# consilience-dev/llm-map-reduce-summarizer

Measured on AMD Instinct MI355X. Metric: chunks/sec (whole node) + end-to-end wall-clock, 10h transcript, Llama-3-8B, higher is better.
Workload: dtype bf16

## Files before the change

### llm_map_reduce_summarizer_amd/csrc/kernels/norm.hip

```cpp
#include "common.h"

template <int VPT, bool ADD, int Q8 = 0>
__global__ __launch_bounds__(256) void rmsnorm_kernel(const bf16* __restrict__ x, bf16* __restrict__ residual,
                                                      const bf16* __restrict__ w, bf16* __restrict__ out,
                                                      int D, int x_stride, int out_stride, float eps,
                                                      float* __restrict__ qscale = nullptr) {
    __shared__ float red[16];
    const int row = blockIdx.x;
    const int nvec = D >> 3;
    const uint4* xr = reinterpret_cast<const uint4*>(x + (size_t)row * x_stride);
    uint4* rr = ADD ? reinterpret_cast<uint4*>(residual + (size_t)row * D) : nullptr;
    float v[VPT][8];
    const uint4* wr = reinterpret_cast<const uint4*>(w);
    uint4 wv[VPT];
#pragma unroll
    for (int i = 0; i < VPT; ++i) wv[i] = wr[min((int)threadIdx.x + i * 256, nvec - 1)];
    float ss = 0.f;
#pragma unroll
    for (int i = 0; i < VPT; ++i) {
        const int c = threadIdx.x + i * 256;
        if (c < nvec) {
            unpack8(xr[c], v[i]);
            if (ADD) {
                float r[8];
                unpack8(rr[c], r);
#pragma unroll
                for (int j = 0; j < 8; ++j) v[i][j] = (float)(bf16)(v[i][j] + r[j]);
                rr[c] = pack8(v[i]);
            }
#pragma unroll
            for (int j = 0; j < 8; ++j) ss += v[i][j] * v[i][j];
        }
    }
    ss = block_sum(ss, red);
    const float inv = rsqrtf(ss / (float)D + eps);
    float amax = 0.f;
#pragma unroll
    for (int i = 0; i < VPT; ++i) {
        const int c = threadIdx.x + i * 256;
        if (c < nvec) {
            float wf[8];
            unpack8(wv[i], wf);
#pragma unroll
            for (int j = 0; j < 8; ++j) v[i][j] = v[i][j] * inv * wf[j];
            if constexpr (Q8) {
#pragma unroll
                for (int j = 0; j < 8; ++j) amax = fmaxf(amax, fabsf(v[i][j]));
            } else {
                reinterpret_cast<uint4*>(out + (size_t)row * out_stride)[c] = pack8(v[i]);
            }
        }
    }
    if constexpr (Q8) {
        amax = wave_max(amax);
        __syncthreads();
        if ((threadIdx.x & 63) == 0) red[threadIdx.x >> 6] = amax;
        __syncthreads();
        amax = fmaxf(fmaxf(red[0], red[1]), fmaxf(red[2], red[3]));
        const float sc = fmaxf(amax, 1e-12f) / 448.f, qi = 1.f / sc;
        if (threadIdx.x == 0) qscale[row] = sc;
        uint2* qr = reinterpret_cast<uint2*>(reinterpret_cast<uint8_t*>(out) + (size_t)row * out_stride);
#pragma unroll
        for (int i = 0; i < VPT; ++i) {
            const int c = threadIdx.x + i * 256;
            if (c < nvec) {
                float y[8];
#pragma unroll
                for (int j = 0; j < 8; ++j) y[j] = v[i][j] * qi;
                int lo = 0, hi = 0;
                lo = __builtin_amdgcn_cvt_pk_fp8_f32(y[0], y[1], lo, false);
                lo = __builtin_amdgcn_cvt_pk_fp8_f32(y[2], y[3], lo, true);
                hi = __builtin_amdgcn_cvt_pk_fp8_f32(y[4], y[5], hi, false);
                hi = __builtin_amdgcn_cvt_pk_fp8_f32(y[6], y[7], hi, true);
                qr[c] = make_uint2((unsigned)lo, (unsigned)hi);
                if constexpr (Q8 == 2) {
                    float r[8];
                    const auto a0 = __builtin_amdgcn_cvt_pk_f32_fp8(lo, false), a1 = __builtin_amdgcn_cvt_pk_f32_fp8(lo, true);
                    const auto b0 = __builtin_amdgcn_cvt_pk_f32_fp8(hi, false), b1 = __builtin_amdgcn_cvt_pk_f32_fp8(hi, true);
                    r[0] = (y[0] - a0[0]) * 16.f; r[1] = (y[1] - a0[1]) * 16.f;
                    r[2] = (y[2] - a1[0]) * 16.f; r[3] = (y[3] - a1[1]) * 16.f;
                    r[4] = (y[4] - b0[0]) * 16.f; r[5] = (y[5] - b0[1]) * 16.f;
                    r[6] = (y[6] - b1[0]) * 16.f; r[7] = (y[7] - b1[1]) * 16.f;
                    int l2 = 0, h2 = 0;
                    l2 = __builtin_amdgcn_cvt_pk_fp8_f32(r[0], r[1], l2, false);
                    l2 = __builtin_amdgcn_cvt_pk_fp8_f32(r[2], r[3], l2, true);
                    h2 = __builtin_amdgcn_cvt_pk_fp8_f32(r[4], r[5], h2, false);
                    h2 = __builtin_amdgcn_cvt_pk_fp8_f32(r[6], r[7], h2, true);
                    qr[nvec + c] = make_uint2((unsigned)l2, (unsigned)h2);
                }
            }
        }
    }
}

template <bool ADD, int Q8 = 0>
static int launch_rmsnorm(const void* x, void* residual, const void* w, void* out, int T, int D, int x_stride,
                          int out_stride, float eps, hipStream_t s, float* qscale = nullptr) {
    if (T <= 0) return 0;
    if (D % 8 || D > 256 * 8 * 8 || (Q8 && !qscale)) return (int)hipErrorInvalidValue;
    const int vpt = ceil_div(D / 8, 256);
    dim3 g(T), b(256);
    auto X = (const bf16*)x; auto R = (bf16*)residual; auto W = (const bf16*)w; auto O = (bf16*)out;
    if (vpt <= 1) rmsnorm_kernel<1, ADD, Q8><<<g, b, 0, s>>>(X, R, W, O, D, x_stride, out_stride, eps, qscale);
    else if (vpt <= 2) rmsnorm_kernel<2, ADD, Q8><<<g, b, 0, s>>>(X, R, W, O, D, x_stride, out_stride, eps, qscale);
    else if (vpt <= 4) rmsnorm_kernel<4, ADD, Q8><<<g, b, 0, s>>>(X, R, W, O, D, x_stride, out_stride, eps, qscale);
    else rmsnorm_kernel<8, ADD, Q8><<<g, b, 0, s>>>(X, R, W, O, D, x_stride, out_stride, eps, qscale);
    return (int)hipGetLastError();
}

MRSUM_API int mrsum_rmsnorm_fp8(const void* x, void* residual, const void* w, void* q, float* qscale, int T, int D,
                                int x_stride, int ldq, float eps, int split, hipStream_t s) {
    if (split) {
        if (ldq < 2 * D) return (int)hipErrorInvalidValue;
        if (residual) return launch_rmsnorm<true, 2>(x, residual, w, q, T, D, x_stride, ldq, eps, s, qscale);
        return launch_rmsnorm<false, 2>(x, nullptr, w, q, T, D, x_stride, ldq, eps, s, qscale);
    }
    if (residual) return launch_rmsnorm<true, 1>(x, residual, w, q, T, D, x_stride, ldq, eps, s, qscale);
    return launch_rmsnorm<false, 1>(x, nullptr, w, q, T, D, x_stride, ldq, eps, s, qscale);
}

MRSUM_API int mrsum_rmsnorm(const void* x, const void* w, void* out, int T, int D, int x_stride, int out_stride,
                            float eps, hipStream_t s) {
    return launch_rmsnorm<false>(x, nullptr, w, out, T, D, x_stride, out_stride, eps, s);
}

MRSUM_API int mrsum_add_rmsnorm(const void* x, void* residual, const void* w, void* out, int T, int D,
                                int x_stride, int out_stride, float eps, hipStream_t s) {
    return launch_rmsnorm<true>(x, residual, w, out, T, D, x_stride, out_stride, eps, s);
}

template <int VPT>
__global__ __launch_bounds__(256) void add_rmsnorm_parts_kernel(const float* __restrict__ parts, int S,
                                                                bf16* __restrict__ residual,
                                                                const bf16* __restrict__ w, bf16* __restrict__ out,
                                                                int T, int D, int out_stride, float eps) {
    __shared__ float red[16];
    const int row = blockIdx.x;
    const int nvec = D >> 3;
    uint4* rr = reinterpret_cast<uint4*>(residual + (size_t)row * D);
    float v[VPT][8];
    float ss = 0.f;
    const uint4* wr = reinterpret_cast<const uint4*>(w);
    uint4 wv[VPT];
#pragma unroll
    for (int i = 0; i < VPT; ++i) wv[i] = wr[min((int)threadIdx.x + i * 256, nvec - 1)];
    uint4 rv[VPT];
    float4 a[VPT][4], bq[VPT][4];
#pragma unroll
    for (int i = 0; i < VPT; ++i) {
        const int c = min((int)threadIdx.x + i * 256, nvec - 1);
        rv[i] = rr[c];
#pragma unroll
        for (int u = 0; u < 4; ++u) {
            const float4* p = reinterpret_cast<const float4*>(parts + ((size_t)min(u, S - 1) * T + row) * D + c * 8);
            a[i][u] = p[0];
            bq[i][u] = p[1];
        }
    }
#pragma unroll
    for (int i = 0; i < VPT; ++i) {
        const int c = threadIdx.x + i * 256;
        unpack8(rv[i], v[i]);
#pragma unroll
        for (int u = 0; u < 4; ++u) {
            if (u < S) {
                v[i][0] += a[i][u].x; v[i][1] += a[i][u].y; v[i][2] += a[i][u].z; v[i][3] += a[i][u].w;
                v[i][4] += bq[i][u].x; v[i][5] += bq[i][u].y; v[i][6] += bq[i][u].z; v[i][7] += bq[i][u].w;
            }
        }
        if (c < nvec) {
            for (int s0 = 4; s0 < S; s0 += 4) {
                float4 x0[4], x1[4];
#pragma unroll
                for (int u = 0; u < 4; ++u) {
                    const float4* p = reinterpret_cast<const float4*>(
                        parts + ((size_t)min(s0 + u, S - 1) * T + row) * D + c * 8);
                    x0[u] = p[0];
                    x1[u] = p[1];
                }
#pragma unroll
                for (int u = 0; u < 4; ++u) {
                    if (s0 + u < S) {
                        v[i][0] += x0[u].x; v[i][1] += x0[u].y; v[i][2] += x0[u].z; v[i][3] += x0[u].w;
                        v[i][4] += x1[u].x; v[i][5] += x1[u].y; v[i][6] += x1[u].z; v[i][7] += x1[u].w;
                    }
                }
            }
#pragma unroll
            for (int j = 0; j < 8; ++j) v[i][j] = (float)(bf16)v[i][j];
            rr[c] = pack8(v[i]);
#pragma unroll
            for (int j = 0; j < 8; ++j) ss += v[i][j] * v[i][j];
        }
    }
    ss = block_sum(ss, red);
    const float inv = rsqrtf(ss / (float)D + eps);
    uint4* orow = reinterpret_cast<uint4*>(out + (size_t)row * out_stride);
#pragma unroll
    for (int i = 0; i < VPT; ++i) {
        const int c = threadIdx.x + i * 256;
        if (c < nvec) {
            float wf[8];
            unpack8(wv[i], wf);
#pragma unroll
            for (int j = 0; j < 8; ++j) v[i][j] = v[i][j] * inv * wf[j];
            orow[c] = pack8(v[i]);
        }
    }
}

MRSUM_API int mrsum_add_rmsnorm_parts(const void* parts, int S, void* residual, const void* w, void* out, int T,
                                      int D, int out_stride, float eps, hipStream_t s) {
    if (T <= 0) return 0;
    if (D % 8 || D > 256 * 8 * 8 || S < 1) return (int)hipErrorInvalidValue;
    const int vpt = ceil_div(D / 8, 256);
    auto P = (const float*)parts; auto R = (bf16*)residual; auto W = (const bf16*)w; auto O = (bf16*)out;
    if (vpt <= 1) add_rmsnorm_parts_kernel<1><<<T, 256, 0, s>>>(P, S, R, W, O, T, D, out_stride, eps);
    else if (vpt <= 2) add_rmsnorm_parts_kernel<2><<<T, 256, 0, s>>>(P, S, R, W, O, T, D, out_stride, eps);
    else if (vpt <= 4) add_rmsnorm_parts_kernel<4><<<T, 256, 0, s>>>(P, S, R, W, O, T, D, out_stride, eps);
    else add_rmsnorm_parts_kernel<8><<<T, 256, 0, s>>>(P, S, R, W, O, T, D, out_stride, eps);
    return (int)hipGetLastError();
}
```

### llm_map_reduce_summarizer_amd/csrc/kernels/sampler.hip

```cpp
#include "common.h"

constexpr int EOS_SLOTS = 4;

__device__ __forceinline__ unsigned long long mix64(unsigned long long x) {
    x ^= x >> 30; x *= 0xbf58476d1ce4e5b9ULL;
    x ^= x >> 27; x *= 0x94d049bb133111ebULL;
    x ^= x >> 31;
    return x;
}

__device__ __forceinline__ unsigned int order_key(float v) {
    const unsigned int b = __float_as_uint(v);
    return (b & 0x80000000u) ? ~b : (b | 0x80000000u);
}

constexpr int FILTER_BINS = 65536;
constexpr int FILTER_R = 4;
constexpr int FILTER_SLICE = FILTER_BINS / FILTER_R;
constexpr int HIST_THREADS = 1024;
constexpr int SELECT_THREADS = 1024;
constexpr int SELECT_CHUNK = FILTER_BINS / SELECT_THREADS;
constexpr int FILTER_CHUNKS = FILTER_BINS / SELECT_CHUNK;
constexpr int FILTER_ROW = FILTER_BINS + FILTER_CHUNKS;

__device__ __forceinline__ int key16(unsigned int h) {
    if ((h & 0x7fffu) > 0x7f80u) return -1;
    if (h == 0x8000u) h = 0u;
    return (int)((h & 0x8000u) ? (~h & 0xffffu) : (h | 0x8000u));
}

__device__ __forceinline__ float key16_value(int key) {
    const unsigned int h = key >= 0x8000 ? ((unsigned int)key & 0x7fffu) : (~(unsigned int)key & 0xffffu);
    return bf16_bits_to_f32(h);
}

__device__ __forceinline__ float level_weight(int key, int top_key, float v1, float inv_tau) {
    return key == top_key ? 1.f : __expf((key16_value(key) - v1) * inv_tau);
}

__device__ __forceinline__ bool filter_active(float tau, int k, float p) { return tau > 0.f && (k > 0 || p < 1.f); }

__global__ __launch_bounds__(HIST_THREADS) void filter_hist_kernel(const bf16* __restrict__ logits, int ld, int V,
                                                                   const float* __restrict__ temps,
                                                                   const int* __restrict__ top_k,
                                                                   const float* __restrict__ top_p,
                                                                   const int* __restrict__ done,
                                                                   unsigned int* __restrict__ hist) {
    __shared__ unsigned int bins[FILTER_SLICE];
    const int b = blockIdx.y;
    if (!filter_active(temps[b], top_k[b], top_p[b]) || done[b]) return;
    const int k0 = blockIdx.x * FILTER_SLICE;
    uint4* bins4 = reinterpret_cast<uint4*>(bins);
    for (int i = threadIdx.x; i < FILTER_SLICE / 4; i += HIST_THREADS) bins4[i] = make_uint4(0u, 0u, 0u, 0u);
    __syncthreads();
    const bf16* row = logits + (size_t)b * ld;
    const unsigned short* rbits = reinterpret_cast<const unsigned short*>(row);
    for (int c = threadIdx.x * 8; c < V; c += HIST_THREADS * 8) {
        unsigned int h[8];
        if (c + 8 <= V) {
            const uint4 v = *reinterpret_cast<const uint4*>(row + c);
            h[0] = v.x & 0xffffu; h[1] = v.x >> 16; h[2] = v.y & 0xffffu; h[3] = v.y >> 16;
            h[4] = v.z & 0xffffu; h[5] = v.z >> 16; h[6] = v.w & 0xffffu; h[7] = v.w >> 16;
        } else {
#pragma unroll
            for (int j = 0; j < 8; ++j) h[j] = c + j < V ? (unsigned int)rbits[c + j] : 0x7fffu;
        }
#pragma unroll
        for (int j = 0; j < 8; ++j) {
            const unsigned int rel = (unsigned int)(key16(h[j]) - k0);
            if (rel < (unsigned int)FILTER_SLICE) atomicAdd(&bins[rel], 1u);
        }
    }
    __syncthreads();
    unsigned int* hrow = hist + (size_t)b * FILTER_ROW;
    uint4* out4 = reinterpret_cast<uint4*>(hrow + k0);
    for (int i = threadIdx.x; i < FILTER_SLICE / 4; i += HIST_THREADS) out4[i] = bins4[i];
    if (threadIdx.x < FILTER_SLICE / SELECT_CHUNK) {
        unsigned int t = 0;
#pragma unroll 8
        for (int i = 0; i < SELECT_CHUNK; ++i)
            t += bins[threadIdx.x * SELECT_CHUNK + ((i + threadIdx.x) & (SELECT_CHUNK - 1))];
        hrow[FILTER_BINS + k0 / SELECT_CHUNK + threadIdx.x] = t;
    }
}

__device__ __forceinline__ void select_scan(int cnt, float mass, int* s_cnt, float* s_mass, int& ex_cnt,
                                            float& ex_mass, int& tot_cnt) {
    const int lane = threadIdx.x & 63, wid = threadIdx.x >> 6;
    int ic = cnt;
    float im = mass;
#pragma unroll
    for (int o = 1; o < 64; o <<= 1) {
        const int oc = __shfl_up(ic, o, 64);
        const float om = __shfl_up(im, o, 64);
        if (lane >= o) { ic += oc; im = om + im; }
    }
    if (lane == 63) { s_cnt[wid] = ic; s_mass[wid] = im; }
    __syncthreads();
    int pc = 0, tc = 0;
    float pm = 0.f;
    for (int w = 0; w < SELECT_THREADS / 64; ++w) {
        if (w < wid) { pc += s_cnt[w]; pm += s_mass[w]; }
        tc += s_cnt[w];
    }
    const float prev = __shfl_up(im, 1, 64);
    ex_cnt = pc + ic - cnt;
    ex_mass = lane == 0 ? pm : pm + prev;
    tot_cnt = tc;
    __syncthreads();
}

__device__ __forceinline__ int block_max_int(int v, int* red) {
#pragma unroll
    for (int o = 32; o > 0; o >>= 1) v = max(v, __shfl_xor(v, o, 64));
    if ((threadIdx.x & 63) == 0) red[threadIdx.x >> 6] = v;
    __syncthreads();
    int m = red[0];
    for (int w = 1; w < SELECT_THREADS / 64; ++w) m = max(m, red[w]);
    __syncthreads();
    return m;
}

__global__ __launch_bounds__(SELECT_THREADS) void filter_select_kernel(const unsigned int* __restrict__ hist, int V,
                                                                       const float* __restrict__ temps,
                                                                       const int* __restrict__ top_k,
                                                                       const float* __restrict__ top_p,
                                                                       const int* __restrict__ done,
                                                                       float* __restrict__ thresh) {
    __shared__ int s_cnt[SELECT_THREADS / 64];
    __shared__ float s_mass[SELECT_THREADS / 64];
    __shared__ int s_red[SELECT_THREADS / 64];
    __shared__ int s_jk;
    __shared__ float s_z;
    const int b = blockIdx.x;
    const float tau = temps[b];
    const int k = top_k[b];
    const float p = top_p[b];
    if (!filter_active(tau, k, p) || done[b]) {
        if (threadIdx.x == 0) thresh[b] = -INFINITY;
        return;
    }
    const int lo = FILTER_BINS - SELECT_CHUNK * ((int)threadIdx.x + 1);
    unsigned int n[SELECT_CHUNK];
    const unsigned int* hrow = hist + (size_t)b * FILTER_ROW;
    const uint4* src = reinterpret_cast<const uint4*>(hrow + lo);
    const bool any = hrow[FILTER_BINS + lo / SELECT_CHUNK] != 0u;
#pragma unroll
    for (int i = 0; i < SELECT_CHUNK / 4; ++i) {
        const uint4 v = any ? src[i] : make_uint4(0u, 0u, 0u, 0u);
        n[4 * i] = v.x; n[4 * i + 1] = v.y; n[4 * i + 2] = v.z; n[4 * i + 3] = v.w;
    }
    int cnt = 0, top = -1;
#pragma unroll
    for (int i = 0; i < SELECT_CHUNK; ++i) {
        cnt += (int)n[i];
        if (n[i]) top = lo + i;
    }
    const int top_key = block_max_int(top, s_red);
    if (top_key < 0) {
        if (threadIdx.x == 0) thresh[b] = -INFINITY;
        return;
    }
    const float v1 = key16_value(top_key);
    const float inv_tau = 1.f / tau;
    float mass = 0.f;
#pragma unroll
    for (int i = SELECT_CHUNK - 1; i >= 0; --i) {
        const int key = lo + i;
        if (n[i]) mass += (float)n[i] * level_weight(key, top_key, v1, inv_tau);
    }
    int ex_cnt, tot;
    float ex_mass;
    select_scan(cnt, mass, s_cnt, s_mass, ex_cnt, ex_mass, tot);
    const int k_eff = (k <= 0 || k >= V) ? tot : min(k, tot);
    if (ex_cnt < k_eff && k_eff <= ex_cnt + cnt) {
        int c = ex_cnt, jk = -1;
        float m = ex_mass, z = 0.f;
#pragma unroll
        for (int i = SELECT_CHUNK - 1; i >= 0; --i) {
            const int key = lo + i;
            if (n[i] && jk < 0) {
                c += (int)n[i];
                m += (float)n[i] * level_weight(key, top_key, v1, inv_tau);
                if (c >= k_eff) { jk = key; z = m; }
            }
        }
        s_jk = jk;
        s_z = z;
    }
    __syncthreads();
    const int jk = s_jk;
    int cut = jk;
    if (p < 1.f) {
        const float target = p * s_z;
        int cand = -1;
        float m = ex_mass;
#pragma unroll
        for (int i = SELECT_CHUNK - 1; i >= 0; --i) {
            const int key = lo + i;
            if (n[i] && key >= jk && cand < 0) {
                m += (float)n[i] * level_weight(key, top_key, v1, inv_tau);
                if (m >= target) cand = key;
            }
        }
        cand = block_max_int(cand, s_red);
        if (cand >= 0) cut = cand;
    }
    if (threadIdx.x == 0) thresh[b] = key16_value(cut);
}

template <bool FILTER>
__global__ __launch_bounds__(256) void sample_kernel(const bf16* __restrict__ logits, int ld, int V, int tok_offset,
                                                     const float* __restrict__ temps,
                                                     const long long* __restrict__ seeds,
                                                     const int* __restrict__ positions,
                                                     unsigned long long* __restrict__ result, int seg_len,
                                                     const float* __restrict__ thresh) {
    __shared__ unsigned long long red[4];
    const int b = blockIdx.y;
    const float tau = temps[b];
    float th = -INFINITY;
    if constexpr (FILTER) th = thresh[b];
    const float inv_tau = tau > 0.f ? 1.f / tau : 0.f;
    const unsigned long long key0 =
        mix64((unsigned long long)seeds[b] * 0x9E3779B97F4A7C15ULL + (unsigned long long)(positions[b] + 1));
    const int c0 = blockIdx.x * seg_len;
    const int c1 = min(V, c0 + seg_len);
    const bf16* row = logits + (size_t)b * ld;
    unsigned long long best = 0;
    for (int c = c0 + threadIdx.x * 8; c < c1; c += 256 * 8) {
        float f[8];
        if (c + 8 <= c1) {
            unpack8(*reinterpret_cast<const uint4*>(row + c), f);
        } else {
#pragma unroll
            for (int j = 0; j < 8; ++j) f[j] = c + j < c1 ? (float)row[c + j] : -INFINITY;
        }
#pragma unroll
        for (int j = 0; j < 8; ++j) {
            const int tok = tok_offset + c + j;
            float v = f[j];
            if constexpr (FILTER) {
                if (v < th) continue;
            }
            if (tau > 0.f) {
                const unsigned long long h = mix64(key0 ^ ((unsigned long long)tok * 0xD1B54A32D192ED03ULL));
                const float u = ((float)(h >> 40) + 0.5f) * (1.f / 16777216.f);
                v = v * inv_tau - __logf(-__logf(u));
            }
            const unsigned long long k =
                ((unsigned long long)order_key(v) << 32) | (unsigned long long)(0xFFFFFFFFu - (unsigned int)tok);
            if (c + j < c1 && k > best) best = k;
        }
    }
#pragma unroll
    for (int o = 32; o > 0; o >>= 1) {
        const unsigned long long other = __shfl_xor(best, o, 64);
        best = other > best ? other : best;
    }
    if ((threadIdx.x & 63) == 0) red[threadIdx.x >> 6] = best;
    __syncthreads();
    if (threadIdx.x == 0) {
        unsigned long long m = red[0];
        for (int i = 1; i < 4; ++i) m = red[i] > m ? red[i] : m;
        atomicMax(result + b, m);
    }
}

__global__ void sample_finish_kernel(unsigned long long* __restrict__ result, int* __restrict__ next_ids,
                                     int* __restrict__ positions, int* __restrict__ gen_count,
                                     const int* __restrict__ max_new, int* __restrict__ out_tokens, int out_stride,
                                     int* __restrict__ done, const int* __restrict__ eos, int B) {
    const int b = blockIdx.x * blockDim.x + threadIdx.x;
    if (b >= B) return;
    const unsigned long long r = result[b];
    result[b] = 0ULL;
    if (done[b]) return;
    const int tok = (int)(0xFFFFFFFFu - (unsigned int)(r & 0xFFFFFFFFULL));
    const int g = gen_count[b];
    out_tokens[(size_t)b * out_stride + g] = tok;
    gen_count[b] = g + 1;
    next_ids[b] = tok;
    bool stop = g + 1 >= max_new[b];
#pragma unroll
    for (int i = 0; i < EOS_SLOTS; ++i) stop |= tok == eos[i];
    if (stop) done[b] = 1;
    else positions[b] += 1;
}

static int launch_keys(const void* logits, int ld, int B, int V, int tok_offset, const float* temps,
                       const long long* seeds, const int* positions, void* result, hipStream_t s) {
    const int nseg = 32;
    int seg_len = ceil_div(V, nseg);
    seg_len = (seg_len + 7) & ~7;
    sample_kernel<false><<<dim3(nseg, B), 256, 0, s>>>((const bf16*)logits, ld, V, tok_offset, temps, seeds,
                                                       positions, (unsigned long long*)result, seg_len, nullptr);
    return (int)hipGetLastError();
}

MRSUM_API int mrsum_sample_keys(const void* logits, int ld, int B, int V, int tok_offset, const float* temps,
                                const long long* seeds, const int* positions, void* result, hipStream_t s) {
    if (B <= 0) return 0;
    return launch_keys(logits, ld, B, V, tok_offset, temps, seeds, positions, result, s);
}

MRSUM_API int mrsum_sample_finish(void* result, int* next_ids, int* positions_rw, int* gen_count, const int* max_new,
                                  int* out_tokens, int out_stride, int* done, const int* eos, int B,
                                  hipStream_t s) {
    if (B <= 0) return 0;
    sample_finish_kernel<<<ceil_div(B, 64), 64, 0, s>>>((unsigned long long*)result, next_ids, positions_rw,
                                                        gen_count, max_new, out_tokens, out_stride, done, eos, B);
    return (int)hipGetLastError();
}

MRSUM_API int mrsum_sample(const void* logits, int ld, int B, int V, const float* temps, const long long* seeds,
                           const int* positions, void* result, int* next_ids, int* positions_rw, int* gen_count,
                           const int* max_new, int* out_tokens, int out_stride, int* done, const int* eos,
                           hipStream_t s) {
    if (B <= 0) return 0;
    int e = launch_keys(logits, ld, B, V, 0, temps, seeds, positions, result, s);
    if (e) return e;
    sample_finish_kernel<<<ceil_div(B, 64), 64, 0, s>>>((unsigned long long*)result, next_ids, positions_rw,
                                                        gen_count, max_new, out_tokens, out_stride, done, eos, B);
    return (int)hipGetLastError();
}

MRSUM_API int mrsum_sample_thresh(const void* logits, int ld, int B, int V, const float* temps, const int* top_k,
                                  const float* top_p, const int* done, float* thresh, void* hist, hipStream_t s) {
    if (B <= 0) return 0;
    filter_hist_kernel<<<dim3(FILTER_R, B), HIST_THREADS, 0, s>>>((const bf16*)logits, ld, V, temps, top_k, top_p,
                                                                  done, (unsigned int*)hist);
    int e = (int)hipGetLastError();
    if (e) return e;
    filter_select_kernel<<<B, SELECT_THREADS, 0, s>>>((const unsigned int*)hist, V, temps, top_k, top_p, done,
                                                      thresh);
    return (int)hipGetLastError();
}

MRSUM_API int mrsum_sample_filtered(const void* logits, int ld, int B, int V, const float* temps,
                                    const long long* seeds, const int* positions, const int* top_k,
                                    const float* top_p, float* thresh, void* hist, void* result, int* next_ids,
                                    int* positions_rw, int* gen_count, const int* max_new, int* out_tokens,
                                    int out_stride, int* done, const int* eos, hipStream_t s) {
    if (B <= 0) return 0;
    int e = mrsum_sample_thresh(logits, ld, B, V, temps, top_k, top_p, done, thresh, hist, s);
    if (e) return e;
    const int nseg = 32;
    int seg_len = ceil_div(V, nseg);
    seg_len = (seg_len + 7) & ~7;
    sample_kernel<true><<<dim3(nseg, B), 256, 0, s>>>((const bf16*)logits, ld, V, 0, temps, seeds, positions,
                                                      (unsigned long long*)result, seg_len, thresh);
    e = (int)hipGetLastError();
    if (e) return e;
    sample_finish_kernel<<<ceil_div(B, 64), 64, 0, s>>>((unsigned long long*)result, next_ids, positions_rw,
                                                        gen_count, max_new, out_tokens, out_stride, done, eos, B);
    return (int)hipGetLastError();
}
```

### llm_map_reduce_summarizer_amd/csrc/kernels/stream_gemm.hip

```cpp
#include "ar_common.h"

namespace {
enum { EPI_BF16 = 0, EPI_F32_PARTIAL = 1, EPI_SWIGLU = 2, EPI_SWIGLU_SPLIT = 3, EPI_RESID_SPLIT = 4 };
constexpr int SS_PARTS = 8;
constexpr int KBLK = 128;
constexpr int LDS_XTRA = 3 * 1024;
constexpr int LDS_BUDGET = 160 * 1024 - LDS_XTRA;

struct NormArgs {
    const float* ssq;
    int ssq_tiles;
    float inv_k, eps;
    bf16* resid;
    int ldr;
    float* ssp;
    int slab_m;
    mrsum_ar::TPPush tp;
};

template <int N>
__device__ __forceinline__ void wait_vmcnt() {
    static_assert(N >= 0 && N < 64, "vmcnt range");
    __builtin_amdgcn_s_waitcnt((N & 15) | (7 << 4) | (15 << 8) | ((N >> 4) << 14));
}

__device__ __forceinline__ void raw_barrier() {
    asm volatile("" ::: "memory");
    __builtin_amdgcn_s_barrier();
    asm volatile("" ::: "memory");
}

__device__ __forceinline__ int img_off(int row, int chunk) {
    return (((row >> 3) << 1) + (chunk >> 3)) * 1024 + ((row & 7) << 7) + ((((chunk & 7) ^ (row & 7))) << 4);
}

template <int AUX = 0>
__device__ __forceinline__ void glds16(const void* g, char* lds) {
    __builtin_amdgcn_global_load_lds((const __attribute__((address_space(1))) void*)g,
                                     (__attribute__((address_space(3))) void*)lds, 16, 0, AUX);
}

__device__ __forceinline__ void row_norm_partials(const NormArgs& e, int M, int tid, int nthr, float* s_ss) {
    const int C = e.ssq_tiles / SS_PARTS;
    for (int i = tid; i < SS_PARTS * M; i += nthr) {
        const int m = i / SS_PARTS, p = i % SS_PARTS;
        const float4* src = reinterpret_cast<const float4*>(e.ssq + (size_t)m * e.ssq_tiles + p * C);
        float4 a = make_float4(0.f, 0.f, 0.f, 0.f);
#pragma unroll 8
        for (int q = 0; q < C / 4; ++q) {
            const float4 v = src[q];
            a.x += v.x; a.y += v.y; a.z += v.z; a.w += v.w;
        }
        s_ss[i] = (a.x + a.y) + (a.z + a.w);
    }
}

__device__ __forceinline__ float row_scale(const NormArgs& e, const float* s_ss, int m) {
    float t = 0.f;
#pragma unroll
    for (int p = 0; p < SS_PARTS; ++p) t += s_ss[SS_PARTS * m + p];
    return rsqrtf(t * e.inv_k + e.eps);
}

__device__ __forceinline__ bool last_arrival(int* counters, int tile, int nsplit, int tid, int* s_flag) {
    asm volatile("s_waitcnt vmcnt(0)" ::: "memory");
    __syncthreads();
    if (tid == 0) {
        const int prev = __hip_atomic_fetch_add(counters + tile, 1, __ATOMIC_RELAXED, __HIP_MEMORY_SCOPE_AGENT);
        *s_flag = prev == nsplit - 1;
    }
    __syncthreads();
    const bool last = *s_flag != 0;
    __builtin_amdgcn_fence(__ATOMIC_ACQUIRE, "wavefront");
    return last;
}

__device__ __forceinline__ void rearm(int* counters, int tile, int tid) {
    if (tid == 0) __hip_atomic_store(counters + tile, 0, __ATOMIC_RELAXED, __HIP_MEMORY_SCOPE_AGENT);
}
}

namespace {
template <int IT, int Q, int NT, int GT>
__device__ __forceinline__ void tp_push_tile(const mrsum_ar::TPPush& tp, float (&h)[IT][4], const uint2 (&rv)[IT],
                                             const int M, const int n0, const int ncols, const int tid,
                                             const unsigned epoch) {
    using namespace mrsum_ar;
#pragma unroll
    for (int j = 0; j < IT; ++j) {
        const int it = tid + j * NT;
        if (it < M * Q)
            tp_push_item(tp, tp_item_off(it / Q, ncols, n0 + 4 * (it % Q)), epoch,
                         make_float4(h[j][0], h[j][1], h[j][2], h[j][3]));
    }
#pragma unroll
    for (int j = 0; j < IT; ++j) {
        const int it = tid + j * NT;
        if (it < M * Q) {
            const float4 acc = tp_gather_item(tp, tp_item_off(it / Q, ncols, n0 + 4 * (it % Q)), epoch);
            h[j][0] = __uint_as_float(rv[j].x << 16) + acc.x;
            h[j][1] = __uint_as_float(rv[j].x & 0xffff0000u) + acc.y;
            h[j][2] = __uint_as_float(rv[j].y << 16) + acc.z;
            h[j][3] = __uint_as_float(rv[j].y & 0xffff0000u) + acc.w;
        }
    }
    if (tid < GT) tp.epochs[n0 / GRAN + tid] = epoch;
}

template <int MT, int EPI, int WPB>
__device__ __forceinline__ void stream_epilogue(f32x4 (&acc)[MT], char* lds, float* s_ss, const int n0, const int M,
                                                void* __restrict__ out, const int ldo, float* __restrict__ parts,
                                                int* __restrict__ counters, const NormArgs& e) {
    const int slab_m = e.slab_m > 0 ? e.slab_m : M;
    constexpr int R = 16 * WPB;
    const int tid = threadIdx.x, lane = tid & 63, w = tid >> 6;
    const int r = lane & 15, g = lane >> 4;
    if (e.ssq) {
        row_norm_partials(e, M, tid, 64 * WPB, s_ss);
        __syncthreads();
#pragma unroll
        for (int m = 0; m < MT; ++m) {
            const float sc = row_scale(e, s_ss, min(16 * m + r, M - 1));
            acc[m][0] *= sc; acc[m][1] *= sc; acc[m][2] *= sc; acc[m][3] *= sc;
        }
    }

    const int nw = n0 + 16 * w;
#pragma unroll
    for (int m = 0; m < MT; ++m) {
        const int mm = 16 * m + r;
        if constexpr (EPI == EPI_SWIGLU) {
            f32x4 up;
#pragma unroll
            for (int jj = 0; jj < 4; ++jj) up[jj] = __shfl_xor(acc[m][jj], 32, 64);
            if (g < 2 && mm < M) {
                float rr[4];
#pragma unroll
                for (int jj = 0; jj < 4; ++jj) {
                    const float gv = acc[m][jj];
                    rr[jj] = gv / (1.f + __expf(-gv)) * up[jj];
                }
                uint2 o;
                o.x = pack2(rr[0], rr[1]);
                o.y = pack2(rr[2], rr[3]);
                *reinterpret_cast<uint2*>(reinterpret_cast<bf16*>(out) + (size_t)mm * ldo + (nw >> 1) + 4 * g) = o;
            }
        } else if (mm < M) {
            if constexpr (EPI == EPI_BF16) {
                uint2 o;
                o.x = pack2(acc[m][0], acc[m][1]);
                o.y = pack2(acc[m][2], acc[m][3]);
                *reinterpret_cast<uint2*>(reinterpret_cast<bf16*>(out) + (size_t)mm * ldo + nw + 4 * g) = o;
            } else if constexpr (EPI == EPI_F32_PARTIAL) {
// ... 124 lines not shown
template <int MT, int EPI, int WPB, bool NTW>
__global__ __launch_bounds__(64 * WPB, 1) void stream_gemm_kernel(const bf16* __restrict__ x, int ldx,
                                                                  const bf16* __restrict__ W, int K, int M,
                                                                  void* __restrict__ out, int ldo, int kper,
                                                                  float* __restrict__ parts, int* __restrict__ counters,
                                                                  const NormArgs e) {
    constexpr int R = 16 * WPB, BM = 16 * MT;
    constexpr int WBYTES = R * 256, SLOT = WBYTES + BM * 256;
    constexpr int D = (LDS_BUDGET / SLOT) < 6 ? (LDS_BUDGET / SLOT) : 6;
    static_assert(D >= 2, "ring too shallow");
    constexpr int XP = 2 * BM / 8;
    constexpr int XI = (XP + WPB - 1) / WPB;
    constexpr int NI = 4 + XI;
    __shared__ __attribute__((aligned(1024))) char lds[D * SLOT + LDS_XTRA];
    float* const s_ss = reinterpret_cast<float*>(lds + D * SLOT + 1024);

    const int tid = threadIdx.x, lane = tid & 63, w = tid >> 6;
    const int n0 = blockIdx.x * R;
    const int ks = blockIdx.y * kper;
    const int nkb = kper / KBLK;

    const int prow = lane >> 3, pslot = lane & 7;
    const bf16* wsrc[4];
#pragma unroll
    for (int p = 0; p < 4; ++p) {
        const int q = 4 * w + p;
        const int row = 8 * (q >> 1) + prow;
        wsrc[p] = W + (size_t)(n0 + row) * K + ks + 8 * (8 * (q & 1) + (pslot ^ prow));
    }
    const bf16* xsrc[XI];
    int xdst[XI];
#pragma unroll
    for (int i = 0; i < XI; ++i) {
        const int q = w + WPB * i;
        const int qq = q < XP ? q : 0;
        const int row = 8 * (qq >> 1) + prow;
        xsrc[i] = x + (size_t)min(row, M - 1) * ldx + ks + 8 * (8 * (qq & 1) + (pslot ^ prow));
        xdst[i] = q < XP ? WBYTES + q * 1024 : -1;
    }
#define ISSUE(slot, kb)                                                                              \
    {                                                                                                \
        char* base = lds + (slot) * SLOT;                                                            \
        _Pragma("unroll") for (int p = 0; p < 4; ++p) glds16<NTW ? 2 : 0>(wsrc[p] + (kb), base + (4 * w + p) * 1024); \
        _Pragma("unroll") for (int i = 0; i < XI; ++i)                                               \
            glds16(xsrc[i] + (kb), xdst[i] >= 0 ? base + xdst[i] : lds + D * SLOT);                  \
    }

    f32x4 acc[MT];
#pragma unroll
    for (int m = 0; m < MT; ++m) acc[m] = f32x4{0.f, 0.f, 0.f, 0.f};

#pragma unroll
    for (int s = 0; s < D - 1; ++s) ISSUE(s, min(s, nkb - 1) * KBLK);

    const int r = lane & 15, g = lane >> 4;
    for (int j = 0; j < nkb; ++j) {
        if (j + D - 2 < nkb) wait_vmcnt<NI * (D - 2)>();
        else wait_vmcnt<0>();
        raw_barrier();
        if (j + D - 1 < nkb) ISSUE((j + D - 1) % D, (j + D - 1) * KBLK);
        const char* wl = lds + (j % D) * SLOT;
        const char* xl = wl + WBYTES;
#pragma unroll
        for (int i = 0; i < 4; ++i) {
            const u32x4 av = *reinterpret_cast<const u32x4*>(wl + img_off(16 * w + r, 4 * i + g));
#pragma unroll
            for (int m = 0; m < MT; ++m) {
                const u32x4 bv = *reinterpret_cast<const u32x4*>(xl + img_off(16 * m + r, 4 * i + g));
                acc[m] = __builtin_amdgcn_mfma_f32_16x16x32_bf16(__builtin_bit_cast(bf16x8, av),
                                                                 __builtin_bit_cast(bf16x8, bv), acc[m], 0, 0, 0);
            }
        }
    }
#undef ISSUE

    stream_epilogue<MT, EPI, WPB>(acc, lds, s_ss, n0, M, out, ldo, parts, counters, e);
}

static bool tp_push_ok(const void* ar, int epi, int M, int N) {
    using namespace mrsum_ar;
    if (!ar) return true;
    auto h = (const ArHandle*)ar;
    if (epi != EPI_RESID_SPLIT || N % GRAN || N / GRAN > MAX_GRAN || (size_t)M * N * 4 > h->max_bytes)
        return false;
    for (int r = 0; r < h->world; ++r)
        if (!h->peers.base[r]) return false;
    return true;
}

MRSUM_API int mrsum_stream_gemm(const void* x, int ldx, const void* W, int N, int K, int M, void* out, int ldo,
                                int epi, int splits, int wpb, void* parts, int* counters, const float* ssq,
                                int ssq_tiles, float eps, void* resid, int ldr, float* ssp, int slab_m, void* ar,
                                hipStream_t s) {
    if (M <= 0) return 0;
    if (wpb < 4 || wpb > 8 || M > 128 || K % KBLK || N % (16 * wpb) || splits < 1 || (K / KBLK) % splits ||
        epi < EPI_BF16 || epi > EPI_RESID_SPLIT)
        return (int)hipErrorInvalidValue;
    if (M > 64 && (ssq || (epi != EPI_BF16 && epi != EPI_F32_PARTIAL && epi != EPI_SWIGLU)))
        return (int)hipErrorInvalidValue;
    if (M > 64) {
        const int slot = (16 * wpb + 16 * (M > 96 ? 8 : 6)) * 256;
        if (LDS_BUDGET / slot < 3) return (int)hipErrorInvalidValue;
    }
    const bool split_epi = epi == EPI_SWIGLU_SPLIT || epi == EPI_RESID_SPLIT;
    if (epi != EPI_F32_PARTIAL && !split_epi && splits != 1) return (int)hipErrorInvalidValue;
    if (split_epi && (!parts || !counters)) return (int)hipErrorInvalidValue;
    if (epi == EPI_RESID_SPLIT && (!resid || !ssp || ldr % 4)) return (int)hipErrorInvalidValue;
    if (ssq && (ssq_tiles <= 0 || ssq_tiles % (4 * SS_PARTS))) return (int)hipErrorInvalidValue;
    if (slab_m && (slab_m < M || epi != EPI_F32_PARTIAL)) return (int)hipErrorInvalidValue;
    if (!tp_push_ok(ar, epi, M, N)) return (int)hipErrorInvalidValue;
    NormArgs e;
    e.ssq = ssq; e.ssq_tiles = ssq_tiles; e.inv_k = 1.f / (float)K; e.eps = eps;
    e.resid = (bf16*)resid; e.ldr = ldr; e.ssp = ssp; e.slab_m = slab_m;
    e.tp = mrsum_ar::tp_push_of((const mrsum_ar::ArHandle*)ar);
    const int kper = K / splits;
    const int mt = (M + 15) / 16;
    dim3 grid(N / (16 * wpb), splits), block(64 * wpb);
    auto X = (const bf16*)x;
    auto Wp = (const bf16*)W;
    auto P = (float*)parts;
#define L(MT_, EPI_, WPB_)                                                                                   \
    stream_gemm_kernel<MT_, EPI_, WPB_, true><<<grid, block, 0, s>>>(X, ldx, Wp, K, M, out, ldo, kper, P, counters, e)
#define BY_WPB(MT_, EPI_)                          \
    switch (wpb) {                                 \
        case 4: L(MT_, EPI_, 4); break;            \
        case 5: L(MT_, EPI_, 5); break;            \
        case 6: L(MT_, EPI_, 6); break;            \
        case 7: L(MT_, EPI_, 7); break;            \
        default: L(MT_, EPI_, 8); break;           \
    }
#define BY_EPI(MT_)                                                           \
    if (epi == EPI_BF16) { BY_WPB(MT_, EPI_BF16) }                            \
    else if (epi == EPI_F32_PARTIAL) { BY_WPB(MT_, EPI_F32_PARTIAL) }         \
    else if (epi == EPI_SWIGLU) { BY_WPB(MT_, EPI_SWIGLU) }                   \
    else if (epi == EPI_SWIGLU_SPLIT) { BY_WPB(MT_, EPI_SWIGLU_SPLIT) }       \
    else { BY_WPB(MT_, EPI_RESID_SPLIT) }
#define BY_EPI_TALL(MT_)                                                      \
    if (epi == EPI_BF16) { BY_WPB(MT_, EPI_BF16) }                            \
    else if (epi == EPI_F32_PARTIAL) { BY_WPB(MT_, EPI_F32_PARTIAL) }         \
    else { BY_WPB(MT_, EPI_SWIGLU) }
    switch (mt) {
        case 1: BY_EPI(1); break;
        case 2: BY_EPI(2); break;
        case 3: BY_EPI(3); break;
        case 4: BY_EPI(4); break;
        case 5: case 6: BY_EPI_TALL(6); break;
        default: BY_EPI_TALL(8); break;
    }
#undef BY_EPI_TALL
#undef BY_EPI
#undef BY_WPB
#undef L
    return (int)hipGetLastError();
}

namespace {
constexpr int KB8 = 256;

__device__ __forceinline__ bf16x8 fp8x8_bf16(uint2 d) {
    typedef __bf16 bf16x2 __attribute__((ext_vector_type(2)));
    const bf16x2 a = __builtin_amdgcn_cvt_scalef32_pk_bf16_fp8(d.x, 1.0f, false);
    const bf16x2 b = __builtin_amdgcn_cvt_scalef32_pk_bf16_fp8(d.x, 1.0f, true);
    const bf16x2 c = __builtin_amdgcn_cvt_scalef32_pk_bf16_fp8(d.y, 1.0f, false);
    const bf16x2 e = __builtin_amdgcn_cvt_scalef32_pk_bf16_fp8(d.y, 1.0f, true);
    return bf16x8{a[0], a[1], b[0], b[1], c[0], c[1], e[0], e[1]};
}
}

constexpr int XR_MAX_K = 8192;

template <int MT, int EPI, int WPB, bool XR>
__global__ __launch_bounds__(64 * WPB, 1) void stream_fp8_kernel(const bf16* __restrict__ x, int ldx,
                                                                 const unsigned char* __restrict__ W,
                                                                 const float* __restrict__ wscale, int K, int M,
                                                                 void* __restrict__ out, int ldo, int kper,
                                                                 float* __restrict__ parts, int* __restrict__ counters,
                                                                 const NormArgs e) {
    constexpr int R = 16 * WPB, BM = 16 * MT;
    constexpr int WBYTES = R * 256, XBYTES = BM * 256, SLOT = XR ? WBYTES : WBYTES + 2 * XBYTES;
    constexpr int XRES = XR ? XR_MAX_K * 2 : 0;
    constexpr int DCAP = XR ? 8 : 6;
    constexpr int D = ((LDS_BUDGET - XRES) / SLOT) < DCAP ? ((LDS_BUDGET - XRES) / SLOT) : DCAP;
    static_assert(D >= 2, "ring too shallow");
    static_assert(!XR || MT == 1, "resident x: one row");
    constexpr int XP = XR ? 0 : 2 * (2 * BM / 8);
    constexpr int XI = (XP + WPB - 1) / WPB;
    constexpr int NI = 4 + XI;
    __shared__ __attribute__((aligned(1024))) char lds[D * SLOT + XRES + LDS_XTRA];
    char* const xres = lds + D * SLOT;
    char* const xtra = lds + D * SLOT + XRES;

    const int tid = threadIdx.x, lane = tid & 63, w = tid >> 6;
    const int n0 = blockIdx.x * R;
    const int ks = blockIdx.y * kper;
    const int nkb = kper / KB8;
    const int prow = lane >> 3, pslot = lane & 7;
    const unsigned char* wsrc[4];
#pragma unroll
    for (int p = 0; p < 4; ++p) {
        const int q = 4 * w + p;
        const int row = 8 * (q >> 1) + prow;
        wsrc[p] = W + (size_t)(n0 + row) * K + ks + 16 * (8 * (q & 1) + (pslot ^ prow));
    }
    constexpr int XPI = 2 * BM / 8;
    const bf16* xsrc[XI > 0 ? XI : 1];
    int xdst[XI > 0 ? XI : 1];
#pragma unroll
    for (int i = 0; i < XI; ++i) {
        const int q = w + WPB * i;
        const int qq = q < XP ? q : 0;
        const int img = qq / XPI, qi = qq % XPI;
        const int row = 8 * (qi >> 1) + prow;
        xsrc[i] = x + (size_t)min(row, M - 1) * ldx + ks + 128 * img + 8 * (8 * (qi & 1) + (pslot ^ prow));
        xdst[i] = q < XP ? WBYTES + img * XBYTES + qi * 1024 : -1;
    }
#define ISSUE8(slot, kb)                                                                             \
    {                                                                                                \
        char* base = lds + (slot) * SLOT;                                                            \
        _Pragma("unroll") for (int p = 0; p < 4; ++p) glds16<2>(wsrc[p] + (kb), base + (4 * w + p) * 1024); \
        _Pragma("unroll") for (int i = 0; i < XI; ++i)                                               \
            glds16(xsrc[i] + (kb), xdst[i] >= 0 ? base + xdst[i] : xtra);                            \
    }
    f32x4 acc[MT];
#pragma unroll
    for (int m = 0; m < MT; ++m) acc[m] = f32x4{0.f, 0.f, 0.f, 0.f};
    if constexpr (XR) {
        for (int p = w; p < kper / 512; p += WPB) glds16(x + ks + 512 * p + 8 * lane, xres + 1024 * p);
    }
#pragma unroll
    for (int s = 0; s < D - 1; ++s) ISSUE8(s, min(s, nkb - 1) * KB8);

    const int r = lane & 15, g = lane >> 4;
    for (int j = 0; j < nkb; ++j) {
        if (j + D - 2 < nkb) wait_vmcnt<NI * (D - 2)>();
        else wait_vmcnt<0>();
        raw_barrier();
        if (j + D - 1 < nkb) ISSUE8((j + D - 1) % D, (j + D - 1) * KB8);
        const char* wl = lds + (j % D) * SLOT;
        const char* xl = wl + WBYTES;
#pragma unroll
        for (int p = 0; p < 4; ++p) {
            const u32x4 a4 = *reinterpret_cast<const u32x4*>(wl + img_off(16 * w + r, 4 * p + g));
#pragma unroll
            for (int h = 0; h < 2; ++h) {
                const bf16x8 av = fp8x8_bf16(make_uint2(a4[2 * h], a4[2 * h + 1]));
                if constexpr (XR) {
                    const u32x4 bv = *reinterpret_cast<const u32x4*>(xres + 2 * (KB8 * j + 64 * p + 16 * g + 8 * h));
                    acc[0] = __builtin_amdgcn_mfma_f32_16x16x32_bf16(av, __builtin_bit_cast(bf16x8, bv), acc[0], 0, 0, 0);
                } else {
#pragma unroll
                    for (int m = 0; m < MT; ++m) {
                        const u32x4 bv = *reinterpret_cast<const u32x4*>(xl + (p >> 1) * XBYTES +
                                                                         img_off(16 * m + r, 8 * (p & 1) + 2 * g + h));
                        acc[m] = __builtin_amdgcn_mfma_f32_16x16x32_bf16(av, __builtin_bit_cast(bf16x8, bv), acc[m], 0, 0, 0);
                    }
                }
            }
        }
    }
#undef ISSUE8

    const float4 sc = *reinterpret_cast<const float4*>(wscale + n0 + 16 * w + 4 * g);
#pragma unroll
    for (int m = 0; m < MT; ++m) {
        acc[m][0] *= sc.x; acc[m][1] *= sc.y; acc[m][2] *= sc.z; acc[m][3] *= sc.w;
    }
    stream_epilogue<MT, EPI, WPB>(acc, lds, reinterpret_cast<float*>(xtra + 1024), n0, M, out, ldo, parts, counters, e);
}

MRSUM_API int mrsum_stream_fp8(const void* x, int ldx, const void* W, const float* wscale, int N, int K, int M,
                               void* out, int ldo, int epi, int splits, int wpb, void* parts, int* counters,
                               const float* ssq, int ssq_tiles, float eps, void* resid, int ldr, float* ssp,
                               void* ar, hipStream_t s) {
    if (M <= 0) return 0;
    if (wpb < 4 || wpb > 8 || M > 64 || K % KB8 || N % (16 * wpb) || splits < 1 || (K / KB8) % splits ||
        epi < EPI_BF16 || epi > EPI_RESID_SPLIT)
        return (int)hipErrorInvalidValue;
    const bool split_epi = epi == EPI_SWIGLU_SPLIT || epi == EPI_RESID_SPLIT;
    if (epi != EPI_F32_PARTIAL && !split_epi && splits != 1) return (int)hipErrorInvalidValue;
    if (split_epi && (!parts || !counters)) return (int)hipErrorInvalidValue;
    if (epi == EPI_RESID_SPLIT && (!resid || !ssp || ldr % 4)) return (int)hipErrorInvalidValue;
    if (ssq && (ssq_tiles <= 0 || ssq_tiles % (4 * SS_PARTS))) return (int)hipErrorInvalidValue;
    if (!tp_push_ok(ar, epi, M, N)) return (int)hipErrorInvalidValue;
    NormArgs e;
    e.ssq = ssq; e.ssq_tiles = ssq_tiles; e.inv_k = 1.f / (float)K; e.eps = eps;
    e.resid = (bf16*)resid; e.ldr = ldr; e.ssp = ssp; e.slab_m = 0;
    e.tp = mrsum_ar::tp_push_of((const mrsum_ar::ArHandle*)ar);
    const int kper = K / splits;
    const int mt = (M + 15) / 16;
    dim3 grid(N / (16 * wpb), splits), block(64 * wpb);
    auto X = (const bf16*)x;
    auto Wp = (const unsigned char*)W;
    auto P = (float*)parts;
    const bool xr = M == 1 && kper <= XR_MAX_K && kper % 512 == 0;
#define L8(MT_, EPI_, WPB_)                                                                                      \
    do {                                                                                                         \
        if (MT_ == 1 && xr)                                                                                      \
            stream_fp8_kernel<1, EPI_, WPB_, true><<<grid, block, 0, s>>>(X, ldx, Wp, wscale, K, M, out, ldo, kper, P, \
                                                                          counters, e);                          \
        else                                                                                                     \
            stream_fp8_kernel<MT_, EPI_, WPB_, false><<<grid, block, 0, s>>>(X, ldx, Wp, wscale, K, M, out, ldo,  \
                                                                             kper, P, counters, e);              \
    } while (0)
#define BY_WPB8(MT_, EPI_)                          \
    switch (wpb) {                                  \
        case 4: L8(MT_, EPI_, 4); break;            \
// ... 23 lines not shown
```

### llm_map_reduce_summarizer_amd/engine/engine.py

```python

from __future__ import annotations

import logging
import os
import time
from dataclasses import dataclass, field, replace
from types import SimpleNamespace
from typing import Dict, List, Optional, Sequence, Tuple

import numpy as np
import torch

from .. import ops
from .config import PREFILL_CHUNK, ModelConfig
from .kv_cache import PagedKVCache
from .model import LlamaModel

log = logging.getLogger("mrsum.engine")

BUCKETS = (1, 2, 4, 8, 16, 24, 32, 40, 48, 64, 80, 96, 128, 160, 192, 224, 256)
MAX_WINDOW = 256
_I32_MAX = 2 ** 31 - 1


# ... 192 lines not shown
            raise ValueError("prefill_chunk must be a multiple of the page size (%d)" % page_size)
        self.sync_every = max(1, sync_every)
        if kv_pages is None:
            if self.device.type == "cuda":
                free, _total = torch.cuda.mem_get_info(self.device)
                budget = int(free * kv_fraction)
            else:
                budget = 256 << 20
            kv_pages = PagedKVCache.size_pages(budget, cfg.n_layers, self.model.hkv, page_size, cfg.head_dim,
                                               kv_dtype=self.kv_dtype)
            kv_pages = min(kv_pages, 1 + self.max_num_seqs * -(-self.max_model_len // page_size))
        self.kv = PagedKVCache(cfg.n_layers, kv_pages, self.model.hkv, page_size, cfg.head_dim, dtype, self.device,
                               kv_dtype=self.kv_dtype)
        self.max_pages = -(-self.max_model_len // page_size)
        self.state = DecodeState(self.max_num_seqs, self.max_pages, max_new_cap, self.device, eos_ids)
        self.pf_tables = torch.zeros(self.max_num_seqs, self.max_pages, dtype=torch.int32, device=self.device)
        self.interleave = os.environ.get("MRSUM_INTERLEAVE", "1") == "1"
        spec = os.environ.get("MRSUM_FAULT_AR_DELAY", "")
        self._fault_delay = tuple(float(x) for x in spec.split(":")) if spec else None
        self.use_graphs = use_graphs and self.device.type == "cuda"
        if self.use_graphs and self.model.tp_size > 1 and self.model.custom_ar is None:
            log.warning("TP=%d without the custom all-reduce: decode hipGraphs disabled", self.model.tp_size)
            self.use_graphs = False
        self._graphs: Dict[tuple, "torch.cuda.CUDAGraph"] = {}
        self._ctx_cls = 0
        self._on_prefill = None
        self._workspaces: Dict[Tuple[int, int], object] = {}
        self.stats = {"prefill_tokens": 0, "prefill_s": 0.0, "decode_steps": 0, "decode_tokens": 0,
                      "decode_s": 0.0, "generate_calls": 0, "graph_captures": 0, "peak_active": 0,
                      "filtered_steps": 0}

    def _bucket(self, n: int) -> int:
        for b in BUCKETS:
            if b >= n:
                return min(b, self.max_num_seqs)
        return self.max_num_seqs

    def _ctx_classes(self) -> int:
        from ..ops.hip import ctx_class
        return ctx_class(self.max_model_len) + 1

    def _workspace(self, B: int):
        if self.device.type != "cuda":
            return None
        key = (B, self._ctx_cls)
        ws = self._workspaces.get(key)
        if ws is None:
            from ..ops.hip import CTX_CLASSES, DecodeWorkspace, decode_attn_plan, decode_groups
            ng = decode_groups(self.model.hq, self.model.hkv)
            s, fused = decode_attn_plan(B, ng, min(CTX_CLASSES[self._ctx_cls], self.max_model_len),
                                        kv8=self.kv.kv_dtype if self.kv.fp8 else False)
            ws = DecodeWorkspace(B, self.model.hq, self.cfg.head_dim, s, self.device, ng, fused_combine=fused)
            self._workspaces[key] = ws
        return ws

    def _sync(self) -> None:
        if self.device.type == "cuda":
            torch.cuda.synchronize(self.device)

    def _prefill(self, seqs: List[_Seq]) -> None:
        chunk = self.prefill_chunk
        if self.model.tp_size > 1 and self.model.sequence_parallel and self.model._sp_backend_ok() and \
                (not chunk or max(len(s.prompt) for s in seqs) <= chunk):
            x = self._pass_inputs(seqs, [(0, len(s.prompt)) for s in seqs], paged=True)
            logits = self.model.prefill_passes([x], self.state.block_tables, self.kv.k, self.kv.v,
                                               gather=self._gather(seqs))
            self.stats["prefill_tokens"] += int(x.ids.numel())
            self._sample_first(seqs, logits)
            return
        if not chunk or max(len(s.prompt) for s in seqs) <= chunk:
            self._prefill_pass(seqs, [(0, len(s.prompt)) for s in seqs], paged=self.paged_prefill)
            return
        rounds = max(-(-len(s.prompt) // chunk) for s in seqs)
        passes = []
        for r in range(rounds):
            k = rounds - 1 - r
            part, spans = [], []
            for s in seqs:
                n = len(s.prompt)
                end = n - k * chunk
                if end > 0:
                    part.append(s)
                    spans.append((max(0, end - chunk), end))
            passes.append((part, spans))
            self.stats["prefill_slices"] = self.stats.get("prefill_slices", 0) + len(part)
        if self.model.tp_size > 1:
            inputs = [self._pass_inputs(part, spans, paged=True) for part, spans in passes]
            logits = self.model.prefill_passes(inputs, self.state.block_tables, self.kv.k, self.kv.v,
                                               gather=self._gather(passes[-1][0]))
            self.stats["prefill_tokens"] += sum(int(x.ids.numel()) for x in inputs)
            self._sample_first(passes[-1][0], logits)
            return
        for r, (part, spans) in enumerate(passes):
            self._prefill_pass(part, spans, paged=True, final=(r == rounds - 1))

    def _pass_inputs(self, seqs: List[_Seq], spans, paged: bool, tables: Optional[torch.Tensor] = None,
                     slots: Optional[List[int]] = None, sample: Optional[List[bool]] = None):
        st, dev = self.state, self.device
        tables = st.block_tables if tables is None else tables
        slots = [s.slot for s in seqs] if slots is None else slots
        lens = [e - b for b, e in spans]
        cu = np.zeros(len(spans) + 1, dtype=np.int32)
        np.cumsum(lens, out=cu[1:])
        ids = np.concatenate([np.asarray(s.prompt[b:e], dtype=np.int32) for s, (b, e) in zip(seqs, spans)])
        pos = np.concatenate([np.arange(b, e, dtype=np.int32) for b, e in spans])
        sidx = np.repeat(np.asarray(slots, dtype=np.int32), lens)
        last = [int(cu[k + 1]) - 1 for k in range(len(spans)) if sample is None or sample[k]]
        h = lambda x: torch.from_numpy(np.ascontiguousarray(x, dtype=np.int32)).to(dev, non_blocking=True)
        items = None
        if dev.type == "cuda":
            from ..ops.hip import prefill_items
            items = prefill_items(lens, self.model.hq // self.model.hkv).to(dev, non_blocking=True)
        pp = None
        if paged:
            pre = [b for b, _ in spans]
            pp = ops.PagedPrefill(tables, h(slots), h(pre), list(slots), pre)
        return SimpleNamespace(ids=h(ids), positions=h(pos), seq_idx=h(sidx), cu_seqlens=h(cu),
                               last_rows=torch.tensor(last, dtype=torch.long).to(dev, non_blocking=True),
                               seqlens=lens, items=items, paged=pp, tables=tables)

    def _sample_first(self, seqs: List[_Seq], logits: torch.Tensor) -> None:
        st = self.state
        v = st.view(seqs[0].slot, len(seqs))
        v.positions.copy_(torch.tensor([len(s.prompt) - 1 for s in seqs], dtype=torch.int32).to(
            self.device, non_blocking=True))
        filtered = _any_filtered(seqs)
        if filtered:
            self.stats["filtered_steps"] += 1
        v.filtered = filtered
        self._sample(logits, v)

    def _gather(self, seqs: Sequence[_Seq]) -> bool:
        return not self.model.tp_sampling or _any_filtered(seqs)

    def _prefill_pass(self, seqs: List[_Seq], spans, paged: bool, final: bool = True) -> None:
        x = self._pass_inputs(seqs, spans, paged)
        logits = self.model.prefill(x.ids, x.positions, x.seq_idx, x.cu_seqlens, x.last_rows, self.state.block_tables,
                                    self.kv.k, self.kv.v, seqlens=x.seqlens, items=x.items,
                                    gather=self._gather(seqs), paged=x.paged, logits=final)
        self.stats["prefill_tokens"] += int(x.ids.numel())
        if final:
            self._sample_first(seqs, logits)

    def _sample(self, logits: torch.Tensor, st_view) -> None:
        if st_view.filtered:
            ops.sample(logits, st_view, filtered=True)
        elif self.model.tp_sampling:
            ops.sample_tp(logits, st_view, self.model.vocab_offset, self.model.custom_ar.max_u64_)
        else:
            ops.sample(logits, st_view)

    def _decode_once(self, B: int, filtered: bool = False) -> None:
        st = self.state
        logits = self.model.decode(st.next_ids[:B], st.positions[:B], st.seq_idx[:B], st.block_tables[:B],
                                   self.kv.k, self.kv.v, workspace=self._workspace(B),
                                   gather=filtered or not self.model.tp_sampling)
        v = st.view(0, B)
        v.filtered = filtered
        self._sample(logits, v)

    def _decode_steps(self, B: int, steps: int, filtered: bool = False) -> None:
        if filtered:
            self.stats["filtered_steps"] += steps
        if self._fault_delay is not None and int(self._fault_delay[0]) == self.model.tp_rank \
                and self.model.custom_ar is not None:
            delay, self._fault_delay = self._fault_delay[1], None
            log.warning("fault injection: TP rank %d sleeps %.1f s before a decode window", self.model.tp_rank, delay)
            time.sleep(delay)
        if not self.use_graphs or (filtered and self.model.tp_sampling):
            for _ in range(steps):
                self._decode_once(B, filtered)
            return
        g = self._graphs.get(self._graph_key(B, filtered))
        if g is None:
            g = self._capture(B, filtered)
        for _ in range(steps):
            g.replay()

    def _graph_key(self, B: int, filtered: bool) -> tuple:
        return (B, self._ctx_cls, True) if filtered else (B, self._ctx_cls)

    def capture_graphs(self, max_batch: Optional[int] = None) -> int:
        if not self.use_graphs:
            return 0
        n = 0
        keep = self._ctx_cls
        try:
            for B in BUCKETS:
                if B > min(max_batch or self.max_num_seqs, self.max_num_seqs):
                    break
                for cls in range(self._ctx_classes() if B == 1 else 1):
                    self._ctx_cls = cls
                    if (B, cls) not in self._graphs:
                        self._capture(B)
                        n += 1
        finally:
            self._ctx_cls = keep
        self._sync()
        return n

    def _capture(self, B: int, filtered: bool = False):
        st = self.state
        snap = {f: getattr(st, f)[:B].clone() for f in DecodeState._ROW_FIELDS}
        s = torch.cuda.Stream(self.device)
        s.wait_stream(torch.cuda.current_stream(self.device))
        with torch.cuda.stream(s):
            self._decode_once(B, filtered)
        torch.cuda.current_stream(self.device).wait_stream(s)
        for f, t in snap.items():
            getattr(st, f)[:B].copy_(t)
        g = torch.cuda.CUDAGraph()
        with torch.cuda.graph(g):
            self._decode_once(B, filtered)
        for f, t in snap.items():
            getattr(st, f)[:B].copy_(t)
        self._graphs[self._graph_key(B, filtered)] = g
        self.stats["graph_captures"] += 1
        return g

    def generate(self, prompts: Sequence[Sequence[int]], params: Sequence[SamplingParams],
                 ignore_eos: bool = False, imported: Optional[Dict[int, ImportedPrefill]] = None,
                 on_prefill=None, feeder=None, on_sync=None) -> List[GenOutput]:
        if len(prompts) != len(params):
            raise ValueError("prompts and params differ in length")
        for sp in params:
            sp.validate()
        eos = list(self.state.eos_ids)
        if ignore_eos:
            self.state.set_eos([])
        try:
            ar = self.model.custom_ar
            failed: Optional[BaseException] = None
            try:
                out = self._generate(prompts, params, imported or {}, on_prefill, feeder, on_sync)
            except Exception as e:
                failed = e
            if ar is not None:
                ar_err, any_failed = ar.agree_error(failed is not None)
                if any_failed:
                    ar.reset()
                if failed is None and any_failed:
                    raise RuntimeError("a tensor-parallel peer failed during this generate")
                if failed is None and ar_err:
                    out = self._recover_custom_ar(prompts, params, imported or {}, on_prefill, feeder, on_sync)
            if failed is not None:
                raise failed
        finally:
            if ignore_eos:
                self.state.set_eos(eos)
        return out

    def _recover_custom_ar(self, prompts, params, imported, on_prefill, feeder, on_sync) -> List[GenOutput]:
        if feeder is not None or on_sync is not None:
            raise RuntimeError("custom all-reduce: a wait for a peer timed out during a streamed generate")
        ar = self.model.custom_ar
        log.error("custom all-reduce: a wait for a peer timed out (TP rank %d); resetting the P2P buffers and "
                  "re-running %d requests on RCCL", self.model.tp_rank, len(prompts))
        self.stats["custom_ar_recoveries"] = self.stats.get("custom_ar_recoveries", 0) + 1
        ar.reset()
        graphs = self.use_graphs
        self.model.custom_ar, self.use_graphs = None, False
        try:
            out = self._generate(prompts, params, imported, on_prefill, None, None)
        finally:
            self.model.custom_ar, self.use_graphs = ar, graphs
        return out

    def _new_seq(self, i: int, p: Sequence[int], sp: SamplingParams, imported=None) -> _Seq:
        p = list(p)
        if not p:
            raise ValueError("empty prompt")
        mn = max(1, min(sp.max_new_tokens, self.max_new_cap))
        if len(p) + mn > self.max_model_len:
            raise ValueError("prompt of %d tokens + %d new exceeds max_model_len %d"
                             % (len(p), mn, self.max_model_len))
        if max(p) >= self.cfg.vocab_size or min(p) < 0:
            raise ValueError("token id out of range")
        sp.validate()
        return _Seq(i, p, replace(sp, max_new_tokens=mn), imported=imported)

    def _fit_ctx_class(self, seqs: Sequence[_Seq]) -> None:
        if seqs and self.device.type == "cuda":
            from ..ops.hip import ctx_class
            self._ctx_cls = max(self._ctx_cls, ctx_class(max(len(s.prompt) + s.params.max_new_tokens for s in seqs)))

    def _generate(self, prompts: Sequence[Sequence[int]], params: Sequence[SamplingParams],
                  imported: Dict[int, ImportedPrefill], on_prefill, feeder=None, on_sync=None) -> List[GenOutput]:
        self.stats["generate_calls"] += 1
        self._on_prefill = on_prefill
        results: List[Optional[GenOutput]] = [None] * len(prompts)
        finished: List[int] = []
        waiting: List[_Seq] = []
        for i, (p, sp) in enumerate(zip(prompts, params)):
            s = self._new_seq(i, p, sp, imported.get(i))
            if s.imported is not None:
                tok = int(s.imported.first_token)
                mn = s.params.max_new_tokens
                if mn == 1 or tok in self.state.eos_ids:
                    results[i] = GenOutput([tok], len(s.prompt), "length" if mn == 1 else "stop")
                    finished.append(i)
                    continue
            waiting.append(s)
        waiting.sort(key=lambda s: -(len(s.prompt) + s.params.max_new_tokens))
        self._ctx_cls = 0
        self._fit_ctx_class(waiting)
        active: List[_Seq] = []
        st = self.state
        if feeder is not None and finished:
            self._feed(feeder, finished, results, waiting)
        prefilling: List[_Seq] = []
        t_window_end = None
        while waiting or active or prefilling:
# ... 380 lines not shown
```

### llm_map_reduce_summarizer_amd/engine/model.py

```python

from __future__ import annotations

import hashlib
import math
import os
from dataclasses import dataclass
from typing import Callable, List, Optional

import torch

from .. import ops
from ..ops.reference import Fp8Weight, interleave_gate_up, rope_cos_sin
from ..parallel.dist import AsyncWorks
from .config import ModelConfig


def _seed_for(seed: int, name: str) -> int:
    return int.from_bytes(hashlib.sha1(("%d:%s" % (seed, name)).encode()).digest()[:8], "little") & ((1 << 63) - 1)


def _randn(shape, std: float, seed: int, name: str, device, dtype) -> torch.Tensor:
    g = torch.Generator(device=device)
    g.manual_seed(_seed_for(seed, name))
    t = torch.randn(*shape, generator=g, device=device, dtype=torch.float32 if device.type == "cpu" else dtype)
    t.mul_(std)
    return t.to(dtype)


class _TPReduce:

    def __init__(self, model: "LlamaModel"):
        self.model = model
        ar = model.custom_ar
        self.fused = ar is not None and os.environ.get("MRSUM_FUSED_AR", "1") == "1"

    def __call__(self, t: torch.Tensor) -> torch.Tensor:
        return self.model._all_reduce(t)

    def fused_ok(self, rows: int, hidden: int) -> bool:
        ar = self.model.custom_ar
        return self.fused and ar is not None and ar.paths["fused_norm"] and rows <= ar.MAX_ROWS and \
            hidden % 4 == 0 and hidden <= 8192 and rows * hidden * 2 <= ar.max_bytes

    def add_rmsnorm(self, parts, residual, ln, eps):
        return self.model.custom_ar.add_rmsnorm(parts, residual, ln, eps)

    def push_ok(self, rows: int, hidden: int) -> bool:
        ar = self.model.custom_ar
        return ar is not None and _tp_push_enabled() and ar.push_ok(rows, hidden)

    def push_handle(self) -> int:
        return self.model.custom_ar.push_handle()

    def push_kinds(self) -> set:
        return self.model.custom_ar.push_kinds()


def _page_of(kcache: torch.Tensor, head_dim: int) -> int:
    if kcache.dtype == torch.uint8:
        return kcache.shape[3] // (head_dim + 4)
    return kcache.shape[3]


_QKV_SPLIT = os.environ.get("MRSUM_FP8_QKV_SPLIT", "1") == "1"


def _hip():
    from ..ops import hip
    return hip


def _tp_push_enabled() -> bool:
    return os.environ.get("MRSUM_TP_PUSH", "1") == "1"


class LocalReduce:
    fused = True

    def __init__(self, model: "LlamaModel"):
        self.model = model

    def __call__(self, t: torch.Tensor) -> torch.Tensor:
        return t

    def fused_ok(self, rows: int, hidden: int) -> bool:
        return rows <= 64

    def add_rmsnorm(self, parts, residual, ln, eps):
        lp = self.model.local_push()
        if lp.fits_rows(parts):
            return lp.add_rmsnorm(parts, residual, ln, eps)
        return ops.add_rmsnorm_parts(parts, residual, ln, eps)

    def push_ok(self, rows: int, hidden: int) -> bool:
        return _tp_push_enabled() and self.model.local_push().push_ok(rows, hidden)

    def push_handle(self) -> int:
        return self.model.local_push().push_handle()


@dataclass
class LayerWeights:
    ln1: torch.Tensor
    wqkv: torch.Tensor
    wo: torch.Tensor
    ln2: torch.Tensor
    wgu: torch.Tensor
    wdown: torch.Tensor


class LlamaModel:
    def __init__(self, cfg: ModelConfig, device: torch.device, dtype: torch.dtype = torch.bfloat16, seed: int = 0,
                 tp_rank: int = 0, tp_size: int = 1, tp_group=None, weight_dtype: str = "bf16",
                 weights_path: Optional[str] = None):
        if weight_dtype not in ("bf16", "fp8"):
            raise ValueError("weight_dtype must be bf16 or fp8")
        self.weight_dtype = weight_dtype
        if cfg.n_heads % tp_size or cfg.n_kv_heads % tp_size or cfg.ffn % tp_size or cfg.vocab_size % tp_size:
            raise ValueError("%s does not shard over tp=%d" % (cfg.name, tp_size))
        self.cfg, self.device, self.dtype = cfg, torch.device(device), dtype
        self.tp_rank, self.tp_size, self.tp_group = tp_rank, tp_size, tp_group
        self.hq, self.hkv, self.hd = cfg.n_heads // tp_size, cfg.n_kv_heads // tp_size, cfg.head_dim
        self.ffn_local = cfg.ffn // tp_size
        self.vocab_local = cfg.vocab_size // tp_size
        self.scale = 1.0 / math.sqrt(cfg.head_dim)
        if weights_path:
            from .weights import load_hf
            self.layers = [LayerWeights(None, None, None, None, None, None) for _ in range(cfg.n_layers)]
            load_hf(self, weights_path)
        else:
            self._init_weights(seed)
        self.cos_sin = rope_cos_sin(cfg.max_position, cfg.head_dim, cfg.rope_theta, self.device,
                                    scaling=cfg.rope_scaling)
        self.vocab_offset = tp_rank * self.vocab_local
        self.emulate_tp_reduce = False
        self._local_push = None
        self.sequence_parallel = os.environ.get("MRSUM_SP", "1") == "1"
        self.custom_ar = None
        if tp_size > 1 and self.device.type == "cuda" and os.environ.get("MRSUM_CUSTOM_AR", "1") == "1":
            from ..parallel.custom_ar import maybe_custom_all_reduce
            self.custom_ar = maybe_custom_all_reduce(tp_group, shapes=dict(
                hidden=cfg.hidden, k={"o": self.hq * self.hd, "down": self.ffn_local},
                fp8=weight_dtype == "fp8", rows=(1, 16, 64)))

    def _init_weights(self, seed: int) -> None:
        c, dev, dt = self.cfg, self.device, self.dtype
        std = c.init_std
        r, tp, hd = self.tp_rank, self.tp_size, c.head_dim
        ones = lambda: torch.ones(c.hidden, device=dev, dtype=dt)
        self.embed = _randn((c.vocab_size, c.hidden), std, seed, "embed", dev, dt)
        self.layers: List[LayerWeights] = []
        for i in range(c.n_layers):
            wq = _randn((c.n_heads * hd, c.hidden), std, seed, "l%d.wq" % i, dev, dt)
            wk = _randn((c.n_kv_heads * hd, c.hidden), std, seed, "l%d.wk" % i, dev, dt)
            wv = _randn((c.n_kv_heads * hd, c.hidden), std, seed, "l%d.wv" % i, dev, dt)
            qs, ks = self.hq * hd, self.hkv * hd
            wqkv = torch.cat([wq[r * qs:(r + 1) * qs], wk[r * ks:(r + 1) * ks], wv[r * ks:(r + 1) * ks]]).contiguous()
            del wq, wk, wv
            wo = _randn((c.hidden, c.n_heads * hd), std, seed, "l%d.wo" % i, dev, dt)
            wo = wo[:, r * qs:(r + 1) * qs].contiguous()
            f = self.ffn_local
            wg = _randn((c.ffn, c.hidden), std, seed, "l%d.wg" % i, dev, dt)
            wu = _randn((c.ffn, c.hidden), std, seed, "l%d.wu" % i, dev, dt)
            wgu = interleave_gate_up(wg[r * f:(r + 1) * f], wu[r * f:(r + 1) * f]).contiguous()
            del wg, wu
            wd = _randn((c.hidden, c.ffn), std, seed, "l%d.wd" % i, dev, dt)
            wd = wd[:, r * f:(r + 1) * f].contiguous()
            if self.weight_dtype == "fp8":
                wqkv, wo, wgu, wd = (Fp8Weight.quantize(t) for t in (wqkv, wo, wgu, wd))
            self.layers.append(LayerWeights(ones(), wqkv, wo, ones(), wgu, wd))
        self.final_norm = ones()
        lm = _randn((c.vocab_size, c.hidden), std, seed, "lm_head", dev, dt)
        v = self.vocab_local
        self.lm_head = lm[r * v:(r + 1) * v].contiguous()
        del lm
        self._quantize_lm_head()

    def _quantize_lm_head(self) -> None:
        if self.weight_dtype == "fp8" and not isinstance(self.lm_head, Fp8Weight):
            self.lm_head = Fp8Weight.quantize(self.lm_head)

    def weight_bytes(self) -> int:
        def nb(t):
            return t.nbytes() if isinstance(t, Fp8Weight) else t.numel() * t.element_size()
        n = nb(self.embed) + nb(self.lm_head) + nb(self.final_norm)
        for lw in self.layers:
            n += sum(nb(t) for t in (lw.ln1, lw.wqkv, lw.wo, lw.ln2, lw.wgu, lw.wdown))
        return n

    def local_push(self):
        if self._local_push is None:
            from ..parallel.custom_ar import LocalPush
            self._local_push = LocalPush()
        return self._local_push

    def _all_reduce(self, t: torch.Tensor) -> torch.Tensor:
        if self.tp_size > 1:
            if self.custom_ar is not None and self.custom_ar.fits(t):
                self.custom_ar.all_reduce(t)
            else:
                if t.is_cuda and torch.cuda.is_current_stream_capturing():
                    raise RuntimeError("TP all-reduce of %s does not fit the P2P buffers inside a hipGraph "
                                       "capture (lower the decode batch or raise max_bytes)" % (tuple(t.shape),))
                torch.distributed.all_reduce(t, group=self.tp_group)
        return t

    def _all_reduce_async(self, t: torch.Tensor):
        if self.tp_size == 1:
            return None
        if self.custom_ar is not None and self.custom_ar.fits(t):
            self.custom_ar.all_reduce(t)
            return None
        return torch.distributed.all_reduce(t, group=self.tp_group, async_op=True)

    def _sp_backend_ok(self) -> bool:
        return True

    def _sp_host(self) -> bool:
        return self.device.type == "cuda" and torch.distributed.get_backend(self.tp_group) != "nccl"

    def _sp_rows(self, T: int):
        Tp = -(-T // self.tp_size) * self.tp_size
        return Tp, Tp // self.tp_size

    def _sp_shard(self, t: torch.Tensor) -> torch.Tensor:
        T = t.shape[0]
        Tp, Ts = self._sp_rows(T)
        out = torch.zeros(Ts, t.shape[1], dtype=t.dtype, device=t.device)
        lo = self.tp_rank * Ts
        n = max(0, min(T, lo + Ts) - lo)
        if n:
            out[:n] = t[lo:lo + n]
        return out

    def _sp_reduce_scatter_async(self, t: torch.Tensor):
        T = t.shape[0]
        Tp, Ts = self._sp_rows(T)
        if Tp != T:
            t = torch.cat([t, torch.zeros(Tp - T, t.shape[1], dtype=t.dtype, device=t.device)])
        if self._sp_host():
            cpu = torch.empty(Ts, t.shape[1], dtype=t.dtype)
            torch.distributed.reduce_scatter_tensor(cpu, t.contiguous().cpu(), group=self.tp_group)
            return cpu.to(t.device), None
        out = torch.empty(Ts, t.shape[1], dtype=t.dtype, device=t.device)
        h = torch.distributed.reduce_scatter_tensor(out, t.contiguous(), group=self.tp_group, async_op=True)
        return out, h

    def _sp_all_gather(self, shard: torch.Tensor, T: int) -> torch.Tensor:
        if self._sp_host():
            cpu = torch.empty(shard.shape[0] * self.tp_size, shard.shape[1], dtype=shard.dtype)
            torch.distributed.all_gather_into_tensor(cpu, shard.contiguous().cpu(), group=self.tp_group)
            return cpu.to(shard.device)[:T]
        out = torch.empty(shard.shape[0] * self.tp_size, shard.shape[1], dtype=shard.dtype, device=shard.device)
        torch.distributed.all_gather_into_tensor(out, shard.contiguous(), group=self.tp_group)
        return out[:T]

    def _prefill_quant(self, T: int):
        if self.weight_dtype != "fp8" or not self.device.type == "cuda" or T <= max(_hip().STREAM_MAX_M,
                                                                                    _hip().STREAM_MAX_M_SWIGLU):
            return False, False
        return True, ("split" if _QKV_SPLIT else True)

    def _add_norm_q(self, x: torch.Tensor, residual: torch.Tensor, eps: float, quant):
        if quant:
            return ops.QuantRows(*_hip().rmsnorm_fp8(x, ops.unit_gain(residual.shape[1], residual.device), eps,
                                                     residual=residual, split=quant == "split"))
        return ops.add_rmsnorm(x, residual, None, eps)

    def _sp_gather_rows(self, x, T: int):
        if isinstance(x, ops.QuantRows):
            q = self._sp_all_gather(x.q.view(torch.uint8), T).view(torch.float8_e4m3fn)
            sc = self._sp_all_gather(x.scale.view(-1, 1), T).view(-1)
            return ops.QuantRows(q.contiguous(), sc.contiguous())
        return self._sp_all_gather(ops.rows(x), T)

    @property
    def tp_sampling(self) -> bool:
        return self.tp_size > 1 and self.custom_ar is not None

    def _gather_vocab(self, logits: torch.Tensor) -> torch.Tensor:
        if self.tp_size == 1:
            return logits
        B, vl = logits.shape
        if logits.is_cuda and torch.distributed.get_backend(self.tp_group) != "nccl":
            cpu = torch.empty(self.tp_size * B, vl, dtype=logits.dtype)
            torch.distributed.all_gather_into_tensor(cpu, logits.cpu().contiguous(), group=self.tp_group)
            out = cpu.to(logits.device)
            return out.view(self.tp_size, B, vl).permute(1, 0, 2).reshape(B, self.tp_size * vl)
        out = torch.empty(self.tp_size * B, vl, dtype=logits.dtype, device=logits.device)
        torch.distributed.all_gather_into_tensor(out, logits.contiguous(), group=self.tp_group)
        return out.view(self.tp_size, B, vl).permute(1, 0, 2).reshape(B, self.tp_size * vl)

    def run_layers(self, ids: torch.Tensor, positions: torch.Tensor, seq_idx: torch.Tensor,
                   block_tables: torch.Tensor, kcache: torch.Tensor, vcache: torch.Tensor,
                   attention: Callable[[int, torch.Tensor], torch.Tensor], decode: bool = False) -> torch.Tensor:
        c = self.cfg
        residual = ops.embed(ids, self.embed)
        q8 = not decode and self.weight_dtype == "fp8"
        q8qkv = ("split" if _QKV_SPLIT else True) if q8 else False
        x = ops.rmsnorm(residual, None, c.rms_eps, quant=q8qkv)
        page = _page_of(kcache, self.hd)
        ar = _TPReduce(self) if self.tp_size > 1 else (LocalReduce(self) if self.emulate_tp_reduce else None)
        last = len(self.layers) - 1
        for i, lw in enumerate(self.layers):
            qkv = ops.qkv_rope(x, lw.wqkv, positions, seq_idx, block_tables, kcache[i], vcache[i], self.cos_sin,
                               self.hq, self.hkv, self.hd, page, defer=decode)
            a = attention(i, qkv)
            x = ops.proj_add_rmsnorm(a, lw.wo, residual, None, c.rms_eps, "o", ar, quant=q8)
            x = ops.mlp(x, lw.wgu, lw.wdown, residual, c.rms_eps, ar,
                        quant=q8qkv if i < last else False)
        return x

    def logits(self, x: torch.Tensor, gather: bool = True) -> torch.Tensor:
        local = ops.linear(x, self.lm_head)
        return self._gather_vocab(local) if gather else local

    def prefill(self, ids: torch.Tensor, positions: torch.Tensor, seq_idx: torch.Tensor, cu_seqlens: torch.Tensor,
                last_rows: torch.Tensor, block_tables: torch.Tensor, kcache: torch.Tensor, vcache: torch.Tensor,
                seqlens: Optional[List[int]] = None, items: Optional[torch.Tensor] = None,
                gather: bool = True, paged=None, logits: bool = True) -> Optional[torch.Tensor]:
        kw = {}
        if ids.is_cuda:
            kw = {"seqlens": seqlens, "items": items}

        def attention(i, qkv):
            pp = paged.layer(kcache[i], vcache[i]) if paged is not None else None
            return ops.attn_prefill(qkv, cu_seqlens, self.hq, self.hkv, self.hd, self.scale, paged=pp, **kw)

        x = self.run_layers(ids, positions, seq_idx, block_tables, kcache, vcache, attention)
        if not logits:
            return None
        return self.logits(ops.rows(x).index_select(0, last_rows), gather)

    def prefill_passes(self, passes, block_tables: torch.Tensor, kcache: torch.Tensor, vcache: torch.Tensor,
                       gather: bool = True) -> torch.Tensor:
        c = self.cfg
        eps = c.rms_eps
        page = _page_of(kcache, self.hd)
        sp = self.sequence_parallel and self.tp_size > 1 and self._sp_backend_ok()
        st = []
        for p in passes:
            res = ops.embed(p.ids, self.embed)
            T = int(res.shape[0])
            q8, q8qkv = self._prefill_quant(T)
            x = ops.rmsnorm(res, None, eps, quant=q8qkv)
            st.append({"res": self._sp_shard(res) if sp else res, "x": x, "T": T, "q": (q8, q8qkv)})

        def wait(h):
            works.wait(h)

        def reduce_async(s, t, key):
            if sp:
                s[key], s["w"] = self._sp_reduce_scatter_async(t)
            else:
                s[key], s["w"] = t, self._all_reduce_async(t)
            works.add(s["w"])

        def add_norm(s, key, last=False):
            wait(s.pop("w"))
            quant = False if last else s["q"][0 if key == "o" else 1]
            x = self._add_norm_q(s.pop(key), s["res"], eps, quant)
            return self._sp_gather_rows(x, s["T"]) if sp else x

        with AsyncWorks() as works:
            for i, lw in enumerate(self.layers):
                for p, s in zip(passes, st):
                    if "d" in s:
                        s["x"] = add_norm(s, "d")
                    qkv = ops.qkv_rope(s["x"], lw.wqkv, p.positions, p.seq_idx, block_tables, kcache[i],
                                       vcache[i], self.cos_sin, self.hq, self.hkv, self.hd, page)
                    kw = {"seqlens": p.seqlens, "items": p.items} if qkv.is_cuda else {}
                    pp = p.paged.layer(kcache[i], vcache[i]) if p.paged is not None else None
                    a = ops.attn_prefill(qkv, p.cu_seqlens, self.hq, self.hkv, self.hd, self.scale, paged=pp, **kw)
                    reduce_async(s, ops.linear(a, lw.wo), "o")
                for s in st:
                    x = add_norm(s, "o")
                    act = ops.gate_up_swiglu(x, lw.wgu)
                    reduce_async(s, ops.linear(act, lw.wdown), "d")
            last, s = passes[-1], st[-1]
            for t in st[:-1]:
                wait(t.pop("w"))
            x = add_norm(s, "d", last=True)
        return self.logits(x.index_select(0, last.last_rows), gather)

    def prefill_cp(self, passes, block_tables: torch.Tensor, kcache: torch.Tensor, vcache: torch.Tensor,
                   exchange, logits_pass: Optional[int] = None) -> Optional[torch.Tensor]:
        c = self.cfg
        eps = c.rms_eps
        page = _page_of(kcache, self.hd)
        st = []
        for p in passes:
            res = ops.embed(p.ids, self.embed)
            q8, q8qkv = self._prefill_quant(int(res.shape[0]))
            st.append({"res": res, "x": ops.rmsnorm(res, None, eps, quant=q8qkv), "q": (q8, q8qkv)})
        last_layer = len(self.layers) - 1
        with AsyncWorks() as works:
            for i, lw in enumerate(self.layers):
                qkvs, handles = [], []
                for k, (p, s) in enumerate(zip(passes, st)):
                    qkvs.append(ops.qkv_rope(s["x"], lw.wqkv, p.positions, p.seq_idx, block_tables, kcache[i],
                                             vcache[i], self.cos_sin, self.hq, self.hkv, self.hd, page))
                    handles.append(exchange.start(i, k))
                    works.add(handles[-1][2])
                for p, s, qkv, h in zip(passes, st, qkvs, handles):
                    exchange.finish(h, works)
                    kw = {"seqlens": p.seqlens, "items": p.items} if qkv.is_cuda else {}
                    a = ops.attn_prefill(qkv, p.cu_seqlens, self.hq, self.hkv, self.hd, self.scale,
                                         paged=p.paged.layer(kcache[i], vcache[i]), **kw)
                    q8, q8qkv = s["q"]
                    x = ops.proj_add_rmsnorm(a, lw.wo, s["res"], None, eps, "o", None, quant=q8)
                    act = ops.gate_up_swiglu(x, lw.wgu)
                    s["x"] = ops.proj_add_rmsnorm(act, lw.wdown, s["res"], None, eps, "down", None,
                                                  quant=q8qkv if i < last_layer else False)
        if logits_pass is None:
            return None
        p, s = passes[logits_pass], st[logits_pass]
        return self.logits(ops.rows(s["x"]).index_select(0, p.last_rows))

    def decode(self, ids: torch.Tensor, positions: torch.Tensor, seq_idx: torch.Tensor, block_tables: torch.Tensor,
               kcache: torch.Tensor, vcache: torch.Tensor, workspace=None, gather: bool = True) -> torch.Tensor:
        page = _page_of(kcache, self.hd)

        def attention(i, qkv):
            return ops.attn_decode(qkv, kcache[i], vcache[i], block_tables, positions, self.hq, self.hkv, self.hd,
                                   page, self.scale, workspace=workspace)

        x = self.run_layers(ids, positions, seq_idx, block_tables, kcache, vcache, attention, decode=True)
        return self.logits(x, gather)
```

### llm_map_reduce_summarizer_amd/ops/__init__.py

```python

from __future__ import annotations

import torch

from . import reference
from .reference import Fp8Weight

def _use_hip(t) -> bool:
    return t.is_cuda


def _impl(t):
    if _use_hip(t):
        from . import hip
        return hip
    return reference


_UNIT = {}


def unit_gain(hidden, device):
    key = (hidden, str(device))
    t = _UNIT.get(key)
    if t is None:
        t = _UNIT[key] = torch.ones(hidden, dtype=torch.bfloat16, device=device)
    return t


def rmsnorm(x, w, eps, out=None, quant=False):
    if w is None:
        w = unit_gain(x.shape[-1], x.device)
    if quant and out is None and _quant_ok(x):
        from . import hip
        return QuantRows(*hip.rmsnorm_fp8(x, w, eps, split=quant == "split"))
    return _impl(x).rmsnorm(x, w, eps, out)


class NormRows:

    def __init__(self, h, ssq, eps):
        self.h, self.ssq, self.eps = h, ssq, eps

    @property
    def shape(self):
        return self.h.shape

    @property
    def norm(self):
        return (self.ssq, self.eps)

    def materialize(self):
        from . import hip
        return hip.rmsnorm(self.h, unit_gain(self.h.shape[1], self.h.device), self.eps)


class QuantRows:

    def __init__(self, q, scale):
        self.q, self.scale = q, scale

    @property
    def shape(self):
        return self.q.shape

    @property
    def pair(self):
        return (self.q, self.scale)


def rows(x):
    if isinstance(x, QuantRows):
        raise TypeError("QuantRows feed fp8 GEMMs only")
    return x.materialize() if isinstance(x, NormRows) else x


def _quant_ok(x) -> bool:
    if not _use_hip(x):
        return False
    from . import hip
    return x.shape[0] > max(hip.STREAM_MAX_M, hip.STREAM_MAX_M_SWIGLU) and x.shape[1] % 16 == 0


def add_rmsnorm(x, residual, w, eps, out=None):
    if w is None:
        w = unit_gain(residual.shape[-1], residual.device)
    return _impl(x).add_rmsnorm(x, residual, w, eps, out)


def rope_kv(qkv, positions, seq_idx, block_tables, kcache, vcache, cos_sin, hq, hkv, d, page, write_cache=True):
    return _impl(qkv).rope_kv(qkv, positions, seq_idx, block_tables, kcache, vcache, cos_sin, hq, hkv, d, page,
                              write_cache)


def rope_kv_parts(parts, positions, seq_idx, block_tables, kcache, vcache, cos_sin, hq, hkv, d, page):
    return _impl(parts).rope_kv_parts(parts, positions, seq_idx, block_tables, kcache, vcache, cos_sin, hq, hkv, d,
                                      page)


def kv_scatter(rows, page, slot, kcache, vcache):
    return _impl(rows).kv_scatter(rows, page, slot, kcache, vcache)


def swiglu(gu, out=None):
    return _impl(gu).swiglu(gu, out)


def linear(x, w):
    if isinstance(x, NormRows):
        from . import hip
        M, K = x.shape
        if isinstance(w, Fp8Weight):
            if hip.fp8_stream_cfg(M, w.shape[0], K, splits=1) is not None:
                return hip.fp8_linear(x.h, w, norm=x.norm)
        elif hip.linear_takes_norm(M, w.shape[0], K):
            return hip.linear(x.h, w, norm=x.norm)
        x = x.materialize()
    if isinstance(w, Fp8Weight):
        if _use_hip(x):
            from . import hip
            return hip.fp8_linear(x, w)
        return reference.linear(x, w)
    return _impl(x).linear(x, w)


def linear_parts(x, w, splits=None):
    if _use_hip(x):
        from . import hip
        return hip.linear_parts(x, w, splits)
    return reference.linear_parts(x, w, splits or 1)


def linear_swiglu(x, w_gu):
    return _impl(x).linear_swiglu(x, w_gu)


def add_rmsnorm_parts(parts, residual, w, eps, out=None):
    return _impl(residual).add_rmsnorm_parts(parts, residual, w, eps, out)


def embed(ids, table, out=None):
    return _impl(table).embed(ids, table, out)


class PagedPrefill:

    def __init__(self, block_tables, seq_slot, prefix, slot_host, prefix_host, kcache=None, vcache=None):
        self.block_tables, self.seq_slot, self.prefix = block_tables, seq_slot, prefix
        self.slot_host, self.prefix_host = list(slot_host), list(prefix_host)
        self.kcache, self.vcache = kcache, vcache

    def layer(self, kcache, vcache) -> "PagedPrefill":
        return PagedPrefill(self.block_tables, self.seq_slot, self.prefix, self.slot_host, self.prefix_host,
                            kcache, vcache)


def attn_prefill(qkv, cu_seqlens, hq, hkv, d, scale, out=None, paged=None, **kw):
    if _use_hip(qkv):
        from . import hip
        return hip.attn_prefill(qkv, cu_seqlens, hq, hkv, d, scale, out, paged=paged, **kw)
    if paged is not None:
        return reference.attn_prefill_paged(qkv, cu_seqlens, hq, hkv, d, scale, paged, out)
    return reference.attn_prefill(qkv, cu_seqlens, hq, hkv, d, scale, out)


def attn_decode(q, kcache, vcache, block_tables, positions, hq, hkv, d, page, scale, out=None, workspace=None):
    if isinstance(q, QKVParts):
        from . import hip
        return hip.attn_decode_rope(q.parts, q.cos_sin, kcache, vcache, block_tables, positions, hq, hkv, d,
                                    page, scale, out, workspace=workspace)
    if _use_hip(q):
        from . import hip
        return hip.attn_decode(q, kcache, vcache, block_tables, positions, hq, hkv, d, page, scale, out,
                               workspace=workspace)
    return reference.attn_decode(q, kcache, vcache, block_tables, positions, hq, hkv, d, page, scale, out)


def sample(logits, st, filtered=False):
    if _use_hip(logits):
        from . import hip
        return hip.sample(logits, st, filtered=filtered)
    n = logits.shape[0]
    thresh = None
    if filtered:
        st.thresh[:n] = reference.nucleus_threshold(logits, st.temps[:n], st.top_k[:n], st.top_p[:n])
        thresh = st.thresh[:n]
    toks = reference.sample_tokens(logits, st.temps[:n], st.seeds[:n], st.positions[:n], thresh)
    reference.sample_finish(toks, st)


def sample_tp(logits, st, tok_offset, max_reduce):
    from . import hip
    return hip.sample_tp(logits, st, tok_offset, max_reduce)



def _plan_parts(hip, p, x, w, splits):
    if p[0] == "stream":
        if isinstance(x, NormRows):
            return hip.linear_parts(x.h, w, p[2], nt=p[1], kernel="stream", norm=x.norm)
        return hip.linear_parts(x, w, p[2], nt=p[1], kernel="stream")
    x = rows(x)
    if p[0] == "lds":
        return hip.linear_parts(x, w, splits or p[1], kernel="lds")
    return hip.linear_parts(x, w, splits or p[2], nt=p[1])


def _fp8_parts(hip, x, w, role, splits):
    cfg = hip.stream_config_fp8(w.shape[0], w.shape[1], splits=splits, M=x.shape[0])
    if cfg is not None:
        if isinstance(x, NormRows):
            return hip.fp8_linear_parts(x.h, w, cfg[1], stream_wpb=cfg[0], norm=x.norm)
        return hip.fp8_linear_parts(x, w, cfg[1], stream_wpb=cfg[0])
    if x.shape[0] == 1 and splits is None:
        N, K = w.shape
        s = next(s for s in (8, 4, 2, 1) if (K // 128) % s == 0 and (K // s >= 2048 or s == 1)
                 and N // 16 * s <= 4096)
        if isinstance(x, NormRows) and hip.skinny_fp8_takes_norm(1, K, s):
            return hip.fp8_linear_parts(x.h, w, s, 1, norm=x.norm)
        return hip.fp8_linear_parts(rows(x), w, s, 1)
    x = rows(x)
    p = hip.plan(role, x.shape[0], w.shape[0], w.shape[1], stream=False)
    nt = p[1] if p[0] == "skinny" else 1
    s = splits or (p[2] if p[0] == "skinny" else (p[1] if p[0] == "lds" else 1))
    if w.shape[0] % (16 * nt):
        nt = 1
    return hip.fp8_linear_parts(x, w, s, nt)


class QKVParts:

    def __init__(self, parts, positions, seq_idx, block_tables, kcache, vcache, cos_sin, hq, hkv, d, page):
        self.parts, self.positions, self.seq_idx, self.block_tables = parts, positions, seq_idx, block_tables
        self.kcache, self.vcache, self.cos_sin = kcache, vcache, cos_sin
        self.hq, self.hkv, self.d, self.page = hq, hkv, d, page

    def materialize(self):
        from . import hip
        return hip.rope_kv_parts(self.parts, self.positions, self.seq_idx, self.block_tables, self.kcache,
                                 self.vcache, self.cos_sin, self.hq, self.hkv, self.d, self.page)


def _defer_ok(hip, defer, x, hq, hkv, d, page):
    return defer and d == 128 and page == 64 and hq % hkv == 0 and hq // hkv <= 16


def qkv_rope(x, wqkv, positions, seq_idx, block_tables, kcache, vcache, cos_sin, hq, hkv, d, page, defer=False):
    if isinstance(x, QuantRows):
        from . import hip
        qkv = hip.fp8_linear(x.pair, wqkv)
        hip.rope_kv(qkv, positions, seq_idx, block_tables, kcache, vcache, cos_sin, hq, hkv, d, page)
        return qkv
    xt = x.h if isinstance(x, NormRows) else x
    if _use_hip(xt) and isinstance(wqkv, Fp8Weight):
        from . import hip
        if x.shape[0] <= hip.SKINNY_MAX_M:
            parts = _fp8_parts(hip, x, wqkv, "qkv", None)
            if _defer_ok(hip, defer, x, hq, hkv, d, page):
                return QKVParts(parts, positions, seq_idx, block_tables, kcache, vcache, cos_sin, hq, hkv, d, page)
            return hip.rope_kv_parts(parts, positions, seq_idx, block_tables, kcache, vcache, cos_sin, hq, hkv, d,
                                     page)
        qkv = hip.fp8_linear(rows(x), wqkv)
        hip.rope_kv(qkv, positions, seq_idx, block_tables, kcache, vcache, cos_sin, hq, hkv, d, page)
        return qkv
    if _use_hip(xt):
        from . import hip
        p = hip.plan("qkv", x.shape[0], wqkv.shape[0], wqkv.shape[1])
        if p[0] != "gemm":
            parts = _plan_parts(hip, p, x, wqkv, None)
            if _defer_ok(hip, defer, x, hq, hkv, d, page):
                return QKVParts(parts, positions, seq_idx, block_tables, kcache, vcache, cos_sin, hq, hkv, d, page)
            return hip.rope_kv_parts(parts, positions, seq_idx, block_tables, kcache, vcache, cos_sin, hq, hkv,
                                     d, page)
        qkv = hip.gemm(rows(x), wqkv)
        hip.rope_kv(qkv, positions, seq_idx, block_tables, kcache, vcache, cos_sin, hq, hkv, d, page)
        return qkv
    qkv = reference.linear(x, wqkv)
    reference.rope_kv(qkv, positions, seq_idx, block_tables, kcache, vcache, cos_sin, hq, hkv, d, page)
    return qkv


def _fused_ar(all_reduce, rows, hidden):
    f = getattr(all_reduce, "add_rmsnorm", None)
    if f is None or not all_reduce.fused_ok(rows, hidden):
        return None
    return f


DEFER_NORM_MAX_M = 16
TP_PUSH_MAX_M = 64
FP8_SKINNY_PUSH_MAX_K = 1024
FP8_SKINNY_PUSH_MAX_K_M1 = 4096


RESID_FORCE = {}


def _resid_plan(hip, a, w, role, tp=False, force=None):
    M = a.shape[0]
    force = force or RESID_FORCE.get(role)
    if M > (TP_PUSH_MAX_M if tp else DEFER_NORM_MAX_M):
        return None
    N, K = w.shape
    if tp and M > 16:
        if force == "skinny":
            return None
        cfg = (hip.fp8_resid_cfg(M, N, K) if isinstance(w, Fp8Weight) else
               (hip.plan(role, M, N, K)[1:] if hip.plan(role, M, N, K)[0] == "stream" else hip.tp_resid_config(N, K)))
        return None if cfg is None or (N // (16 * cfg[0])) % 32 else ("stream",) + tuple(cfg)
    if isinstance(w, Fp8Weight):
        if force == "skinny" or (force is None and tp and (K <= FP8_SKINNY_PUSH_MAX_K or
                                                           (M == 1 and K <= FP8_SKINNY_PUSH_MAX_K_M1))):
            ok = M <= 16 and N % 512 == 0 and N // 16 <= hip.skinny_fp8_resid_capacity()
            if ok or force == "skinny":
                return ("skinny",) if ok else None
        cfg = hip.fp8_resid_cfg(M, N, K)
    else:
        p = hip.plan(role, M, N, K)
        cfg = p[1:] if p[0] == "stream" else None
        if not tp and M <= 16 and N % 512 == 0 and (force == "skinny" or (force is None and role == "o" and K <= 4096)):
            return ("skinny",)
        if tp:
            if (force == "skinny" or (force is None and p[0] == "skinny")) and N % 512 == 0 \
                    and N // 16 <= hip.skinny_resid_capacity(N):
                return ("skinny",)
            if force == "skinny":
                return None
            if cfg is None or force == "stream":
                cfg = hip.tp_resid_config(N, K)
    if cfg is None or (N // (16 * cfg[0])) % 32:
        return None
    return ("stream",) + tuple(cfg)


def proj_add_rmsnorm(a, w, residual, ln, eps, role="o", all_reduce=None, quant=False):
    if _use_hip(a):
        from . import hip
        if ln is None and a.shape[0] <= hip.SKINNY_MAX_M:
            ok = getattr(all_reduce, "push_ok", None)
            push = all_reduce.push_handle() if ok is not None and ok(a.shape[0], residual.shape[1]) else None
            if all_reduce is None or push is not None:
                rp = _resid_plan(hip, a, w, role, tp=push is not None)
                kinds = getattr(all_reduce, "push_kinds", None)
                if push is not None and rp is not None and kinds is not None and rp[0] not in kinds():
                    other = ({"stream", "skinny"} - {rp[0]}) & kinds()
                    rp = _resid_plan(hip, a, w, role, tp=True, force=other.pop()) if other else None
                if rp is not None and rp[0] == "skinny":
                    return NormRows(residual, hip.skinny_resid(a, w, residual, tp=push), eps)
                if rp is not None:
                    return NormRows(residual, hip.stream_resid(a, w, residual, rp[1], rp[2], tp=push), eps)
    if ln is None:
        ln = unit_gain(residual.shape[1], residual.device)
    if _use_hip(a) and isinstance(w, Fp8Weight):
        from . import hip
        if a.shape[0] <= hip.SKINNY_MAX_M:
            fused = _fused_ar(all_reduce, a.shape[0], residual.shape[1])
            parts = _fp8_parts(hip, a, w, role, 1 if (all_reduce and not fused) else None)
            if fused:
                return fused(parts, residual, ln, eps)
            if all_reduce:
                all_reduce(parts)
            return hip.add_rmsnorm_parts(parts, residual, ln, eps)
        o = hip.fp8_linear(a, w)
        if all_reduce:
            all_reduce(o)
        if quant and _quant_ok(o):
            return QuantRows(*hip.rmsnorm_fp8(o, ln, eps, residual=residual, split=quant == "split"))
        return hip.add_rmsnorm(o, residual, ln, eps)
    if _use_hip(a):
        from . import hip
        fused = _fused_ar(all_reduce, a.shape[0], residual.shape[1])
        one = 1 if (all_reduce and not fused) else None
        p = hip.plan(role, a.shape[0], w.shape[0], w.shape[1], splits=one)
        if p[0] != "gemm":
            parts = _plan_parts(hip, p, a, w, one)
            if fused:
                return fused(parts, residual, ln, eps)
            if all_reduce:
                all_reduce(parts)
            return hip.add_rmsnorm_parts(parts, residual, ln, eps)
        o = hip.gemm(a, w)
        if all_reduce:
            all_reduce(o)
        if quant and _quant_ok(o):
            return QuantRows(*hip.rmsnorm_fp8(o, ln, eps, residual=residual, split=quant == "split"))
        return hip.add_rmsnorm(o, residual, ln, eps)
    o = reference.linear(a, w)
    if all_reduce:
        all_reduce(o)
    return reference.add_rmsnorm(o, residual, ln, eps)


def mlp(x, wgu, wdown, residual, eps, all_reduce=None, quant=False):
    act = gate_up_swiglu(x, wgu)
    return proj_add_rmsnorm(act, wdown, residual, None, eps, "down", all_reduce, quant=quant)


def gate_up_swiglu(x, wgu):
    if isinstance(x, QuantRows):
        from . import hip
        return hip.fp8_linear_swiglu(x.pair, wgu)
    xt = x.h if isinstance(x, NormRows) else x
    if _use_hip(xt) and isinstance(wgu, Fp8Weight):
        from . import hip
        if isinstance(x, NormRows) and hip.fp8_swiglu_takes_norm(x.shape[0], wgu.shape[0], x.shape[1]):
            return hip.fp8_linear_swiglu(x.h, wgu, norm=x.norm)
        return hip.fp8_linear_swiglu(rows(x), wgu)
    if _use_hip(xt):
        from . import hip
        p = hip.plan("gate_up", x.shape[0], wgu.shape[0], wgu.shape[1])
        nr = isinstance(x, NormRows) and p[0] in ("stream", "stream_split", "skinny")
        xin, norm = (x.h, x.norm) if nr else (rows(x), None)
        if p[0] == "stream":
            return hip.linear_swiglu(xin, wgu, kernel="stream", wpb=p[1], norm=norm)
        if p[0] == "stream_split":
            return hip.linear_swiglu(xin, wgu, kernel="stream_split", wpb=p[1], splits=p[2], norm=norm)
        return hip.linear_swiglu(xin, wgu, kernel=p[0], norm=norm)
    return reference.swiglu(reference.linear(x, wgu))
```

### llm_map_reduce_summarizer_amd/ops/hip.py

```python

from __future__ import annotations

import ctypes
import os
from typing import Optional

import torch

from ._lib import kernels_lib
from .reference import Fp8Weight

_c_int, _c_float, _vp = ctypes.c_int, ctypes.c_float, ctypes.c_void_p

_SIGS = {
    "mrsum_rmsnorm": [_vp, _vp, _vp, _c_int, _c_int, _c_int, _c_int, _c_float, _vp],
    "mrsum_add_rmsnorm": [_vp, _vp, _vp, _vp, _c_int, _c_int, _c_int, _c_int, _c_float, _vp],
    "mrsum_rmsnorm_fp8": [_vp, _vp, _vp, _vp, _vp, _c_int, _c_int, _c_int, _c_int, _c_float, _c_int, _vp],
    "mrsum_rope_kv": [_vp, _c_int, _c_int, _vp, _vp, _vp, _c_int, _vp, _vp, _vp, _c_int, _c_int, _c_int, _c_int,
                      _c_int, _c_int, _vp],
    "mrsum_rope_kv_parts": [_vp, _c_int, _vp, _c_int, _c_int, _vp, _vp, _vp, _c_int, _vp, _vp, _vp, _c_int,
                            _c_int, _c_int, _c_int, _c_int, _vp],
    "mrsum_swiglu": [_vp, _vp, _c_int, _c_int, _vp],
    "mrsum_kv_scatter": [_vp, _c_int, _c_int, _c_int, _vp, _vp, _vp, _vp, _c_int, _vp],
    "mrsum_embed": [_vp, _vp, _vp, _c_int, _c_int, _c_int, _vp],
    "mrsum_attn_prefill": [_vp, _c_int, _vp, _vp, _c_int, _c_int, _vp, _c_int, _c_int, _c_int, _c_int, _c_float, _vp],
    "mrsum_attn_prefill_paged": [_vp, _c_int, _vp, _vp, _c_int, _c_int, _vp, _c_int, _c_int, _c_int, _c_int, _c_float,
                                 _vp,
                                 _vp, _vp, _c_int, _vp, _vp, _c_int, _vp],
    "mrsum_attn_decode_mfma": [_vp, _c_int, _vp, _vp, _vp, _c_int, _vp, _vp, _vp, _vp, _c_int, _c_int, _c_int,
                               _c_int, _c_int, _c_int, _c_int, _c_float, _vp, _c_int, _vp],
    "mrsum_attn_decode_rope": [_vp, _c_int, _vp, _vp, _vp, _vp, _c_int, _vp, _vp, _vp, _vp, _c_int, _c_int,
                               _c_int, _c_int, _c_int, _c_int, _c_int, _c_float, _vp, _c_int, _vp],
    "mrsum_skinny_gemm": [_vp, _c_int, _vp, _c_int, _c_int, _c_int, _vp, _c_int, _c_int, _c_int, _c_int, _vp, _c_int,
                          _c_float, _vp, _c_int, _vp, _vp, _c_int, _vp],
    "mrsum_skinny_resid_capacity_w": [_c_int],
    "mrsum_skinny_lds": [_vp, _c_int, _vp, _c_int, _c_int, _c_int, _vp, _c_int, _c_int, _c_int, _c_int, _vp],
    "mrsum_stream_gemm": [_vp, _c_int, _vp, _c_int, _c_int, _c_int, _vp, _c_int, _c_int, _c_int, _c_int, _vp, _vp,
                          _vp, _c_int, _c_float, _vp, _c_int, _vp, _c_int, _vp, _vp],
    "mrsum_stream_fp8": [_vp, _c_int, _vp, _vp, _c_int, _c_int, _c_int, _vp, _c_int, _c_int, _c_int, _c_int, _vp, _vp,
                         _vp, _c_int, _c_float, _vp, _c_int, _vp, _vp, _vp],
    "mrsum_skinny_fp8": [_vp, _c_int, _vp, _vp, _c_int, _c_int, _c_int, _vp, _c_int, _c_int, _c_int, _c_int, _vp,
                         _c_int, _c_float, _vp, _c_int, _vp, _vp, _c_int, _vp],
    "mrsum_skinny_fp8_resid_capacity": [],
    "mrsum_quant_fp8_rows": [_vp, _c_int, _vp, _vp, _c_int, _c_int, _vp],
    "mrsum_add_rmsnorm_parts": [_vp, _c_int, _vp, _vp, _vp, _c_int, _c_int, _c_int, _c_float, _vp],
    "mrsum_sample_keys": [_vp, _c_int, _c_int, _c_int, _c_int, _vp, _vp, _vp, _vp, _vp],
    "mrsum_sample_finish": [_vp, _vp, _vp, _vp, _vp, _vp, _c_int, _vp, _vp, _c_int, _vp],
    "mrsum_gemm": [_vp, _c_int, _vp, _c_int, _vp, _c_int, _c_int, _c_int, _c_int, _c_int, _c_int, _vp, _vp, _c_int,
                   _c_int, _vp],
    "mrsum_sample": [_vp, _c_int, _c_int, _c_int, _vp, _vp, _vp, _vp, _vp, _vp, _vp, _vp, _vp, _c_int, _vp, _vp,
                     _vp],
    "mrsum_sample_thresh": [_vp, _c_int, _c_int, _c_int, _vp, _vp, _vp, _vp, _vp, _vp, _vp],
    "mrsum_sample_filtered": [_vp, _c_int, _c_int, _c_int, _vp, _vp, _vp, _vp, _vp, _vp, _vp, _vp, _vp, _vp, _vp,
                              _vp, _vp, _c_int, _vp, _vp, _vp],
}

_fns = {}


def _fn(name: str):
    f = _fns.get(name)
    if f is None:
        lib = kernels_lib()
        f = getattr(lib, name)
        f.argtypes = _SIGS[name]
        f.restype = ctypes.c_int
        _fns[name] = f
    return f


def _stream() -> int:
    return torch.cuda.current_stream().cuda_stream


def _p(t: Optional[torch.Tensor]) -> Optional[int]:
    return None if t is None else t.data_ptr()


DEBUG_SYNC = os.environ.get("MRSUM_DEBUG_SYNC", "0") == "1"


def _check(rc: int, name: str) -> None:
    if rc != 0:
        raise RuntimeError("%s launch failed: hipError %d" % (name, rc))
    if DEBUG_SYNC and not torch.cuda.is_current_stream_capturing():
        try:
            torch.cuda.synchronize()
        except RuntimeError as e:
            raise RuntimeError("%s: device error after the launch: %s" % (name, e)) from e


def _req(cond: bool, msg: str) -> None:
    if not cond:
        raise ValueError(msg)


def _bf16_cuda(*ts: torch.Tensor) -> None:
    for t in ts:
        _req(t.is_cuda and t.dtype == torch.bfloat16, "expected a bf16 CUDA tensor, got %s %s" % (t.dtype, t.device))


def _i32(*ts: torch.Tensor) -> None:
    for t in ts:
        _req(t.is_cuda and t.dtype == torch.int32 and t.is_contiguous(), "expected a contiguous int32 CUDA tensor")


def _rows_ok(x: torch.Tensor) -> None:
    _req(x.dim() == 2 and x.stride(1) == 1 and x.stride(0) % 8 == 0 and x.data_ptr() % 16 == 0,
         "expected a 2-D row-major tensor with 16-byte aligned rows")


def rmsnorm(x: torch.Tensor, w: torch.Tensor, eps: float, out: Optional[torch.Tensor] = None) -> torch.Tensor:
    _bf16_cuda(x, w)
    _rows_ok(x)
    T, D = x.shape
    _req(w.numel() == D and w.is_contiguous() and D % 8 == 0 and D <= 16384, "rmsnorm: bad weight / D")
    if out is None:
        out = torch.empty(T, D, dtype=x.dtype, device=x.device)
    _rows_ok(out)
    _req(out.shape == (T, D), "rmsnorm: bad out shape")
    _check(_fn("mrsum_rmsnorm")(_p(x), _p(w), _p(out), T, D, x.stride(0), out.stride(0), eps, _stream()),
           "rmsnorm")
    return out


def add_rmsnorm(x: torch.Tensor, residual: torch.Tensor, w: torch.Tensor, eps: float,
                out: Optional[torch.Tensor] = None) -> torch.Tensor:
    _bf16_cuda(x, residual, w)
    _rows_ok(x)
    T, D = x.shape
    _req(residual.shape == (T, D) and residual.is_contiguous(), "add_rmsnorm: residual must be [T, D] contiguous")
    _req(w.numel() == D and D % 8 == 0 and D <= 16384, "add_rmsnorm: bad weight / D")
    if out is None:
        out = torch.empty(T, D, dtype=x.dtype, device=x.device)
    _rows_ok(out)
    _check(_fn("mrsum_add_rmsnorm")(_p(x), _p(residual), _p(w), _p(out), T, D, x.stride(0), out.stride(0), eps,
                                    _stream()), "add_rmsnorm")
    return out


def rmsnorm_fp8(x: torch.Tensor, w: torch.Tensor, eps: float, residual: Optional[torch.Tensor] = None,
                split: bool = False):
    _bf16_cuda(x, w)
    _rows_ok(x)
    T, D = x.shape
    _req(w.numel() == D and w.is_contiguous() and D % 16 == 0 and D <= 16384, "rmsnorm_fp8: bad weight / D")
    if residual is not None:
        _bf16_cuda(residual)
        _req(residual.shape == (T, D) and residual.is_contiguous(), "rmsnorm_fp8: residual must be [T, D] contiguous")
    q = torch.empty(T, 2 * D if split else D, dtype=torch.float8_e4m3fn, device=x.device)
    sc = torch.empty(T, dtype=torch.float32, device=x.device)
    _check(_fn("mrsum_rmsnorm_fp8")(_p(x), _p(residual), _p(w), _p(q), _p(sc), T, D, x.stride(0), q.shape[1], eps,
                                    1 if split else 0, _stream()), "rmsnorm_fp8")
    return q, sc


KV8_PAGE, KV8_D = 64, 128
KV8_SLAB = KV8_PAGE * KV8_D + 4 * KV8_PAGE


def _cache_kind(kcache: torch.Tensor, vcache: torch.Tensor, hkv: int, page: int, d: int, what: str) -> int:
    _req(kcache is not None and vcache is not None and kcache.is_cuda and vcache.is_cuda
         and kcache.is_contiguous() and vcache.is_contiguous() and kcache.shape[0] == vcache.shape[0],
         "%s: K / V caches must be contiguous CUDA tensors with the same pages" % what)
    kind = 0
    for bit, c in ((1, kcache), (2, vcache)):
        if c.dtype == torch.uint8:
            _req(page == KV8_PAGE and d == KV8_D and tuple(c.shape[1:]) == (hkv, KV8_SLAB),
                 "%s: fp8 cache must be uint8 [pages, Hkv, %d] (page 64, head dim 128)" % (what, KV8_SLAB))
            kind |= bit
        else:
            _req(c.dtype == torch.bfloat16 and tuple(c.shape[1:]) == (hkv, page, d),
                 "%s: cache must be bf16 [pages, Hkv, P, D] (or the fp8 slab layout)" % what)
    _req(kind != 1, "%s: an fp8 K cache needs an fp8 V cache (formats: bf16, fp8, fp8v)" % what)
    return kind


def rope_kv(qkv: torch.Tensor, positions: torch.Tensor, seq_idx: torch.Tensor, block_tables: torch.Tensor,
            kcache: Optional[torch.Tensor], vcache: Optional[torch.Tensor], cos_sin: torch.Tensor,
            hq: int, hkv: int, d: int, page: int, write_cache: bool = True, check_bounds: bool = False) -> None:
    _bf16_cuda(qkv)
    _rows_ok(qkv)
    T = qkv.shape[0]
    if T == 0:
        return
    _req(qkv.shape[1] >= (hq + 2 * hkv) * d and d in (64, 128), "rope_kv: qkv too narrow / bad head dim")
    _i32(positions, seq_idx, block_tables)
    _req(positions.numel() >= T and seq_idx.numel() >= T, "rope_kv: positions/seq_idx shorter than T")
    _req(cos_sin.is_cuda and cos_sin.dtype == torch.float32 and cos_sin.is_contiguous()
         and cos_sin.shape[1:] == (d // 2, 2), "rope_kv: cos_sin must be [max_pos, D/2, 2] fp32")
    kv8 = 0
    if write_cache:
        kv8 = _cache_kind(kcache, vcache, hkv, page, d, "rope_kv")
        _req(block_tables.dim() == 2, "rope_kv: block_tables must be 2-D")
    if check_bounds:
        pmax = int(positions[:T].max())
        _req(pmax < cos_sin.shape[0], "rope_kv: position %d beyond rope table" % pmax)
        if write_cache:
            _req(pmax // page < block_tables.shape[1], "rope_kv: position beyond block table")
            _req(int(seq_idx[:T].max()) < block_tables.shape[0] and int(seq_idx[:T].min()) >= 0, "rope_kv: seq_idx")
    _check(_fn("mrsum_rope_kv")(_p(qkv), T, qkv.stride(0), _p(positions), _p(seq_idx), _p(block_tables),
                                block_tables.stride(0), _p(kcache) if write_cache else None,
                                _p(vcache) if write_cache else None, _p(cos_sin), hq, hkv, d, page,
                                1 if write_cache else 0, kv8, _stream()), "rope_kv")


def rope_kv_parts(parts: torch.Tensor, positions: torch.Tensor, seq_idx: torch.Tensor, block_tables: torch.Tensor,
                  kcache: torch.Tensor, vcache: torch.Tensor, cos_sin: torch.Tensor, hq: int, hkv: int, d: int,
                  page: int, out: Optional[torch.Tensor] = None) -> torch.Tensor:
    _req(parts.is_cuda and parts.dtype == torch.float32 and parts.is_contiguous() and parts.dim() == 3,
         "rope_kv_parts: parts must be fp32 [S, T, W]")
    S, T, W = parts.shape
    _req(W == (hq + 2 * hkv) * d and d in (64, 128), "rope_kv_parts: width")
    _i32(positions, seq_idx, block_tables)
    _req(positions.numel() >= T and seq_idx.numel() >= T and block_tables.dim() == 2, "rope_kv_parts: tables")
    _req(cos_sin.is_cuda and cos_sin.dtype == torch.float32 and cos_sin.shape[1:] == (d // 2, 2), "cos_sin")
    kv8 = _cache_kind(kcache, vcache, hkv, page, d, "rope_kv_parts")
    if out is None:
        out = torch.empty(T, W, dtype=torch.bfloat16, device=parts.device)
    _rows_ok(out)
    _check(_fn("mrsum_rope_kv_parts")(_p(parts), S, _p(out), T, out.stride(0), _p(positions), _p(seq_idx),
                                      _p(block_tables), block_tables.stride(0), _p(kcache), _p(vcache), _p(cos_sin),
                                      hq, hkv, d, page, kv8, _stream()), "rope_kv_parts")
    return out


def kv_scatter(rows: torch.Tensor, page: torch.Tensor, slot: torch.Tensor, kcache: torch.Tensor,
               vcache: torch.Tensor) -> None:
    _bf16_cuda(rows, kcache, vcache)
    _i32(page, slot)
    n = rows.shape[0]
    _req(rows.is_contiguous() and rows.dim() == 4 and rows.shape[1] == 2 and tuple(rows.shape[2:]) ==
         (kcache.shape[1], kcache.shape[3]), "kv_scatter: rows must be [n, 2, hkv, d]")
    _req(kcache.is_contiguous() and vcache.is_contiguous() and kcache.shape == vcache.shape, "kv_scatter: cache")
    _req(page.numel() >= n and slot.numel() >= n, "kv_scatter: index")
    _check(_fn("mrsum_kv_scatter")(_p(rows), n, kcache.shape[1], kcache.shape[3], _p(page), _p(slot), _p(kcache),
                                   _p(vcache), kcache.shape[2], _stream()), "kv_scatter")


def swiglu(gu: torch.Tensor, out: Optional[torch.Tensor] = None) -> torch.Tensor:
    _bf16_cuda(gu)
    _req(gu.dim() == 2 and gu.is_contiguous() and gu.shape[1] % 32 == 0, "swiglu: gu must be [T, 2F], F % 16 == 0")
    T, F = gu.shape[0], gu.shape[1] // 2
    if out is None:
        out = torch.empty(T, F, dtype=gu.dtype, device=gu.device)
    _req(out.is_contiguous() and out.shape == (T, F), "swiglu: bad out")
    _check(_fn("mrsum_swiglu")(_p(gu), _p(out), T, F, _stream()), "swiglu")
    return out


def embed(ids: torch.Tensor, table: torch.Tensor, out: Optional[torch.Tensor] = None) -> torch.Tensor:
    _i32(ids)
    _bf16_cuda(table)
    _req(table.is_contiguous() and table.shape[1] % 8 == 0, "embed: table must be [V, D] contiguous")
    T = ids.numel()
    V, D = table.shape
    if out is None:
        out = torch.empty(T, D, dtype=table.dtype, device=table.device)
    _req(out.is_contiguous() and out.shape == (T, D), "embed: bad out")
    _check(_fn("mrsum_embed")(_p(ids), _p(table), _p(out), T, D, V, _stream()), "embed")
    return out


def prefill_block_m(group: int) -> int:
    _req(1 <= group <= 64, "attn_prefill: GQA ratio %d out of range" % group)
    return 256 // group if group in (1, 2, 4, 8) else 256


def prefill_items(seqlens, group: int) -> torch.Tensor:
    block_m = prefill_block_m(group)
    items = []
    for s, n in enumerate(seqlens):
        for qb in range(0, int(n), block_m):
            items.append((qb, s))
    items.sort(key=lambda x: -x[0])
    return torch.tensor([(s, qb) for qb, s in items], dtype=torch.int32).reshape(-1, 2)


def attn_prefill(qkv: torch.Tensor, cu_seqlens: torch.Tensor, hq: int, hkv: int, d: int, scale: float,
                 out: Optional[torch.Tensor] = None, items: Optional[torch.Tensor] = None,
                 seqlens=None, paged=None) -> torch.Tensor:
    _bf16_cuda(qkv)
    _rows_ok(qkv)
    _req(d == 128 and hq % hkv == 0 and qkv.shape[1] >= (hq + 2 * hkv) * d, "attn_prefill: bad head config")
    _i32(cu_seqlens)
    T = qkv.shape[0]
    if seqlens is None:
        cu = cu_seqlens.cpu().tolist()
        seqlens = [b - a for a, b in zip(cu[:-1], cu[1:])]
        _req(cu[0] == 0 and cu[-1] <= T and all(n >= 0 for n in seqlens), "attn_prefill: bad cu_seqlens")
    block_m = prefill_block_m(hq // hkv)
    if items is None:
        items = prefill_items(seqlens, hq // hkv).to(qkv.device)
    _req(items.shape[0] == sum(-(-int(n) // block_m) for n in seqlens),
         "attn_prefill: work list not built for GQA ratio %d (prefill_items(seqlens, %d))" % (hq // hkv, hq // hkv))
    _i32(items)
    if out is None:
        out = torch.empty(T, hq * d, dtype=qkv.dtype, device=qkv.device)
    _rows_ok(out)
    _req(out.shape[0] >= T and out.shape[1] >= hq * d, "attn_prefill: bad out")
    if paged is not None:
        kc, vc, bt = paged.kcache, paged.vcache, paged.block_tables
        kv8 = _cache_kind(kc, vc, hkv, 64, d, "attn_prefill")
        _i32(bt, paged.seq_slot, paged.prefix)
        _req(bt.dim() == 2 and len(paged.prefix_host) == len(seqlens) == paged.seq_slot.numel(),
             "attn_prefill: paged tables")
        for pre, n, slot in zip(paged.prefix_host, seqlens, paged.slot_host):
            _req(0 <= slot < bt.shape[0] and pre >= 0 and pre + n <= bt.shape[1] * 64,
                 "attn_prefill: slice [%d, %d) beyond block table" % (pre, pre + n))
        _check(_fn("mrsum_attn_prefill_paged")(_p(qkv), qkv.stride(0), _p(cu_seqlens), _p(items), items.shape[0],
                                               block_m, _p(out), out.stride(0), hq, hkv, d, scale, _p(kc), _p(vc), _p(bt),
                                               bt.stride(0), _p(paged.seq_slot), _p(paged.prefix), kv8, _stream()),
               "attn_prefill_paged")
        return out
    _check(_fn("mrsum_attn_prefill")(_p(qkv), qkv.stride(0), _p(cu_seqlens), _p(items), items.shape[0], block_m, _p(out),
                                     out.stride(0), hq, hkv, d, scale, _stream()), "attn_prefill")
    return out


def decode_splits(batch: int, hkv: int, max_ctx: int, target_wgs: int = 1024, max_splits: int = 32) -> int:
    s = max(1, -(-target_wgs // max(1, batch * hkv)))
    s = min(s, max_splits, max(1, -(-max_ctx // 64)))
    return s


MAX_SPLITS = 256
TP_SHARD_MAX_SPLITS = 128
ATTN_PAGES_PER_SPLIT = 2


CTX_CLASSES = (6144, 12288, 32768, 1 << 30)


def ctx_class(ctx: int) -> int:
    for i, c in enumerate(CTX_CLASSES):
        if ctx <= c:
            return i
    return len(CTX_CLASSES) - 1


ATTN_SLOTS = 768


KV8_SPLIT_GROUPS = 96


def decode_attn_plan(batch: int, hkv: int, max_ctx: int, kv8=False):
    s, fused = decode_attn_plan_bf16(batch, hkv, max_ctx)
    if kv8 is True or kv8 == "fp8":
        mult = 2.0 if batch * hkv <= KV8_SPLIT_GROUPS else 1.0
        pages = max(1, -(-max_ctx // 64))
        s = max(1, min(int(round(s * mult)), pages, 64, 16 if fused else 64))
    return s, fused


def decode_attn_plan_bf16(batch: int, hkv: int, max_ctx: int):
    pages = max(1, -(-max_ctx // 64))
    groups = max(1, batch * hkv)
    splits = max(1, min(ATTN_SLOTS // groups, -(-pages // ATTN_PAGES_PER_SPLIT), 64))
    if pages <= 96:
        splits = max(1, min(max(3, N_CU // groups), -(-pages // ATTN_PAGES_PER_SPLIT), 64))
        if groups >= 256:
            splits = min(4, -(-pages // ATTN_PAGES_PER_SPLIT))
    if groups <= 16:
        fused = -(-pages // 16) <= 6
        if fused and hkv <= 2:
            return max(1, min(N_CU // groups, pages, 64)), False
        if not fused and hkv <= 2:
            return max(1, min(ATTN_SLOTS // groups, -(-pages // ATTN_PAGES_PER_SPLIT), TP_SHARD_MAX_SPLITS)), False
        if fused and batch == 1 and hkv >= 8 and pages > 32:
            fused = False
            splits = min(splits, 32)
        elif fused:
            splits = min(splits, 16)
        elif pages <= 512:
            splits = min(splits, 32)
    else:
        fused = groups <= 128
        if fused:
            if pages <= 96:
                splits = min(splits, 12 if hkv <= 2 else 8)
            else:
                splits = min(splits, 4 if hkv <= 2 else 6)
    return splits, fused


def decode_groups(hq: int, hkv: int) -> int:
    _req(hkv > 0 and hq % hkv == 0 and hq // hkv <= 64, "decode attention: bad head config %d / %d" % (hq, hkv))
    return hkv if hq // hkv in (1, 2, 4, 8, 16) else hq


class DecodeWorkspace:

    def __init__(self, batch: int, hq: int, d: int, splits: int, device, hkv: Optional[int] = None,
                 fused_combine: bool = False):
        self.splits = splits
        self.part_o = torch.empty(batch * hq * splits * d, dtype=torch.float32, device=device)
        self.part_ml = torch.empty(batch * hq * splits * 2, dtype=torch.float32, device=device)
        self.counters = (torch.zeros(batch * (hkv or hq), dtype=torch.int32, device=device)
                         if fused_combine else None)



def attn_decode_rope(parts: torch.Tensor, cos_sin: torch.Tensor, kcache: torch.Tensor, vcache: torch.Tensor,
                     block_tables: torch.Tensor, positions: torch.Tensor, hq: int, hkv: int, d: int, page: int,
                     scale: float, out: Optional[torch.Tensor] = None,
                     workspace: Optional[DecodeWorkspace] = None) -> torch.Tensor:
    _req(parts.is_cuda and parts.dtype == torch.float32 and parts.is_contiguous() and parts.dim() == 3,
         "attn_decode_rope: parts must be fp32 [S, B, width]")
    SP, B, width = parts.shape
    _req(width == (hq + 2 * hkv) * d and d == 128 and page == 64 and hq % hkv == 0 and hq // hkv <= 64,
         "attn_decode_rope: unsupported config")
    ng = decode_groups(hq, hkv)
    kv8 = _cache_kind(kcache, vcache, hkv, page, d, "attn_decode_rope")
# ... 195 lines not shown
    return _gemm(_p(xq), xq.stride(0), _p(q), K, out, M, N, K, 1, GEMM_EPI_SWIGLU if swiglu else GEMM_EPI_BF16,
                 _p(xs), _p(sc), group_m, 1 if split else 0)


SKINNY_MAX_M = 64
STREAM_MAX_M = 256
STREAM_MAX_M_SWIGLU = 128
EPI_BF16, EPI_F32_PARTIAL, EPI_SWIGLU, EPI_SWIGLU_SPLIT, EPI_RESID_SPLIT = 0, 1, 2, 3, 4
EPI_SKINNY_RESID = 3


def choose_splits(N: int, K: int, nt: int, target_wgs: int = 512, max_splits: int = 8) -> int:
    blocks = K // 128
    base = N // (16 * nt)
    for s in range(1, max_splits + 1):
        if blocks % s == 0 and base * s >= target_wgs:
            return s
    best = 1
    for s in range(1, max_splits + 1):
        if blocks % s == 0:
            best = s
    return best


SKINNY_WAVES8_MAX_WGS = 2 * 256
SKINNY_WAVES8_MAX_M = 1
SKINNY_WAVES_FORCE = int(os.environ["MRSUM_SKINNY_WAVES"]) if os.environ.get("MRSUM_SKINNY_WAVES") else None


def skinny_waves(N: int, nt: int, splits: int, M: int = 1) -> int:
    if SKINNY_WAVES_FORCE in (4, 8):
        return SKINNY_WAVES_FORCE
    return 8 if M <= SKINNY_WAVES8_MAX_M and (N // (16 * nt)) * splits <= SKINNY_WAVES8_MAX_WGS else 4


def _skinny(x, w, out, epi, nt, splits, ldo, norm=None, resid=None, ssp=None, ar=None):
    _bf16_cuda(x, w)
    _rows_ok(x)
    M, K = x.shape
    N = w.shape[0]
    _req(w.is_contiguous() and w.shape[1] == K, "skinny_gemm: weight must be [N, K] contiguous")
    _req(1 <= M <= SKINNY_MAX_M and K % 128 == 0 and N % (16 * nt) == 0 and (K // 128) % splits == 0,
         "skinny_gemm: unsupported shape M=%d N=%d K=%d nt=%d S=%d" % (M, N, K, nt, splits))
    sq, tiles, eps = _norm_args(x, norm)
    rp, ldr, sp = None, 0, None
    if epi == EPI_SKINNY_RESID:
        _req(nt == 1 and splits == 1 and M <= 16, "skinny resid: one 16-row tile per workgroup, M <= 16")
        _bf16_cuda(resid)
        _rows_ok(resid)
        _req(resid.shape == (M, N) and ssp is not None and ssp.dtype == torch.float32 and ssp.is_contiguous()
             and ssp.shape == (M, N // 16), "skinny resid: residual [M, N] bf16 and ssp fp32 [M, N / 16]")
        rp, ldr, sp = _p(resid), resid.stride(0), _p(ssp)
    _check(_fn("mrsum_skinny_gemm")(_p(x), x.stride(0), _p(w), N, K, M, _p(out), ldo, epi, nt, splits, sq, tiles, eps,
                                    rp, ldr, sp, ar, skinny_waves(N, nt, splits, M), _stream()), "skinny_gemm")
    return out


def _skinny_lds(x, w, out, epi, splits, ldo, wpb=4):
    _bf16_cuda(x, w)
    _rows_ok(x)
    M, K = x.shape
    N = w.shape[0]
    _req(w.is_contiguous() and w.shape[1] == K, "skinny_lds: weight must be [N, K] contiguous")
    _req(1 <= M <= SKINNY_MAX_M and K % 128 == 0 and 4 <= wpb <= 8 and N % (16 * wpb) == 0
         and (K // 128) % splits == 0, "skinny_lds: unsupported shape M=%d N=%d K=%d S=%d wpb=%d" % (M, N, K, splits, wpb))
    _check(_fn("mrsum_skinny_lds")(_p(x), x.stride(0), _p(w), N, K, M, _p(out), ldo, epi, splits, wpb, _stream()),
           "skinny_lds")
    return out


def _norm_args(x, norm):
    if norm is None:
        return None, 0, 0.0
    ssq, eps = norm
    _req(ssq.is_cuda and ssq.dtype == torch.float32 and ssq.is_contiguous() and ssq.dim() == 2
         and ssq.shape[0] == x.shape[0] and ssq.shape[1] % 32 == 0, "deferred norm: ssq must be fp32 [M, 32k]")
    return _p(ssq), ssq.shape[1], float(eps)


def _resid_args(x, N, epi, resid, ssp):
    if epi != EPI_RESID_SPLIT:
        return None, 0, None
    M = x.shape[0]
    _bf16_cuda(resid)
    _rows_ok(resid)
    _req(resid.shape == (M, N) and ssp is not None and ssp.dtype == torch.float32 and ssp.is_contiguous()
         and ssp.dim() == 2 and ssp.shape[0] == M, "resid split: residual [M, N] bf16 and ssp fp32 [M, tiles]")
    return _p(resid), resid.stride(0), _p(ssp)


def _stream_gemm(x, w, out, epi, splits, ldo, wpb, parts=None, counters=None, norm=None, resid=None, ssp=None,
                 ar=None):
    _bf16_cuda(x, w)
    _rows_ok(x)
    M, K = x.shape
    N = w.shape[0]
    if M > SKINNY_MAX_M and epi in (EPI_BF16, EPI_F32_PARTIAL, EPI_SWIGLU) and norm is None:
        ch = STREAM_TALL_M
        for r0 in range(0, M, ch):
            r1 = min(M, r0 + ch)
            if r1 - r0 > SKINNY_MAX_M:
                tw = tall_wpb(N, r1 - r0, splits)
                if tw is not None:
                    o = out[:, r0:r1] if epi == EPI_F32_PARTIAL else out[r0:r1]
                    _stream_launch(x[r0:r1], w, o, epi, splits, ldo, tw, None, None, None, None, None,
                                   M if epi == EPI_F32_PARTIAL else 0)
                    continue
            for c0 in range(r0, r1, SKINNY_MAX_M):
                c1 = min(r1, c0 + SKINNY_MAX_M)
                o = out[:, c0:c1] if epi == EPI_F32_PARTIAL else out[c0:c1]
                _stream_launch(x[c0:c1], w, o, epi, splits, ldo, wpb, None, None, None, None, None,
                               M if epi == EPI_F32_PARTIAL else 0)
        return out
    return _stream_launch(x, w, out, epi, splits, ldo, wpb, parts, counters, norm, resid, ssp, 0, ar)


STREAM_TALL_M = 128
_TALL_WPB = {6: (4, 5, 6), 8: (4, 5)}


def tall_wpb(N: int, M: int, splits: int) -> Optional[int]:
    mt = 6 if M <= 96 else 8
    best, key = None, None
    for wpb in _TALL_WPB[mt]:
        if N % (16 * wpb):
            continue
        grid = N // (16 * wpb) * splits
        k = (round(grid / (-(-grid // N_CU) * N_CU), 3), wpb)
        if key is None or k > key:
            best, key = wpb, k
    return best


def _stream_launch(x, w, out, epi, splits, ldo, wpb, parts, counters, norm, resid, ssp, slab_m, ar=None):
    M, K = x.shape
    N = w.shape[0]
    _req(w.is_contiguous() and w.shape[1] == K, "stream_gemm: weight must be [N, K] contiguous")
    tall_ok = M <= 128 and epi in (EPI_BF16, EPI_F32_PARTIAL, EPI_SWIGLU) and norm is None
    _req(1 <= M and (M <= SKINNY_MAX_M or tall_ok) and K % 128 == 0 and 4 <= wpb <= 8 and N % (16 * wpb) == 0
         and (K // 128) % splits == 0, "stream_gemm: unsupported shape M=%d N=%d K=%d S=%d wpb=%d"
         % (M, N, K, splits, wpb))
    if epi in (EPI_SWIGLU_SPLIT, EPI_RESID_SPLIT):
        _req(parts is not None and parts.shape == (splits, M, N) and parts.dtype == torch.float32
             and counters is not None and counters.numel() >= N // (16 * wpb), "stream_gemm: split-K scratch")
    if epi == EPI_RESID_SPLIT:
        _req(ssp.shape[1] == N // (16 * wpb), "stream_gemm: ssp tiles")
    sq, tiles, eps = _norm_args(x, norm)
    rp, ldr, sp = _resid_args(x, N, epi, resid, ssp)
    _check(_fn("mrsum_stream_gemm")(_p(x), x.stride(0), _p(w), N, K, M, _p(out), ldo, epi, splits, wpb, _p(parts),
                                    _p(counters), sq, tiles, eps, rp, ldr, sp, slab_m, ar, _stream()), "stream_gemm")
    return out


def linear_takes_norm(M: int, N: int, K: int) -> bool:
    return 1 <= M <= SKINNY_MAX_M and K % 128 == 0 and stream_config(N, K, splits=1) is not None


def linear(x: torch.Tensor, w: torch.Tensor, out: Optional[torch.Tensor] = None, norm=None) -> torch.Tensor:
    M, K = x.shape
    N = w.shape[0]
    _req(norm is None or linear_takes_norm(M, N, K), "linear: a deferred norm needs a stream-GEMM shape")
    tall = (SKINNY_MAX_M < M <= STREAM_TALL_M and K % 128 == 0 and norm is None
            and stream_config(N, K, splits=1) is not None and tall_wpb(N, M, 1) is not None)
    if (M > SKINNY_MAX_M and not tall) or M == 0 or K % 128:
        return gemm(x, w, out=out)
    if out is None:
        out = torch.empty(M, N, dtype=x.dtype, device=x.device)
    _req(out.is_contiguous() and out.shape == (M, N), "linear: bad out")
    if tall:
        return _stream_gemm(x, w, out, EPI_BF16, 1, N, tall_wpb(N, M, 1))
    cfg = stream_config(N, K, splits=1)
    if cfg is not None:
        return _stream_gemm(x, w, out, EPI_BF16, 1, N, cfg[0], norm=norm)
    nt = 2 if N % 32 == 0 and N >= 16384 else 1
    if N % (16 * nt):
        return gemm(x, w, out=out)
    return _skinny(x, w, out, EPI_BF16, nt, 1, N)


def linear_parts(x: torch.Tensor, w: torch.Tensor, splits: Optional[int] = None,
                 out: Optional[torch.Tensor] = None, nt: int = 1, kernel: str = "skinny", norm=None) -> torch.Tensor:
    M, K = x.shape
    N = w.shape[0]
    if splits is None:
        splits = choose_splits(N, K, nt if kernel == "skinny" else 4)
    if out is None:
        out = torch.empty(splits, M, N, dtype=torch.float32, device=x.device)
    _req(out.is_contiguous() and out.shape == (splits, M, N) and out.dtype == torch.float32, "linear_parts: bad out")
    if kernel == "stream":
        return _stream_gemm(x, w, out, EPI_F32_PARTIAL, splits, N, nt, norm=norm)
    _req(norm is None, "linear_parts: a deferred norm needs the stream kernel")
    if kernel == "lds":
        return _skinny_lds(x, w, out, EPI_F32_PARTIAL, splits, N)
    return _skinny(x, w, out, EPI_F32_PARTIAL, nt, splits, N)


_TILE_COUNTERS = {}


def _tile_counters(device, n: int) -> torch.Tensor:
    key = (str(device), n)
    t = _TILE_COUNTERS.get(key)
    if t is None:
        _req(not torch.cuda.is_current_stream_capturing(), "split-K SwiGLU tickets first used inside a capture")
        t = _TILE_COUNTERS[key] = torch.zeros(max(n, 1024), dtype=torch.int32, device=device)
    return t


def stream_swiglu_split(x: torch.Tensor, w_gu: torch.Tensor, out: torch.Tensor, wpb: int, splits: int,
                        norm=None) -> torch.Tensor:
    M, K = x.shape
    N = w_gu.shape[0]
    _req(out.is_contiguous() and out.shape == (M, N // 2), "stream_swiglu_split: bad out")
    parts = torch.empty(splits, M, N, dtype=torch.float32, device=x.device)
    cnt = _tile_counters(x.device, N // (16 * wpb))
    return _stream_gemm(x, w_gu, out, EPI_SWIGLU_SPLIT, splits, out.stride(0), wpb, parts=parts, counters=cnt,
                        norm=norm)


def stream_resid(x: torch.Tensor, w, residual: torch.Tensor, wpb: int, splits: int, tp=None) -> torch.Tensor:
    M = x.shape[0]
    fp8 = isinstance(w, Fp8Weight)
    N = (w.q if fp8 else w).shape[0]
    tiles = N // (16 * wpb)
    if tp is not None:
        STATS["tp_push"] += 1
    parts = torch.empty(splits, M, N, dtype=torch.float32, device=x.device)
    ssp = torch.empty(M, tiles, dtype=torch.float32, device=x.device)
    cnt = _tile_counters(x.device, tiles)
    if fp8:
        _stream_fp8(x, w, None, EPI_RESID_SPLIT, splits, 0, wpb, parts=parts, counters=cnt, resid=residual, ssp=ssp,
                    ar=tp)
    else:
        _stream_gemm(x, w, None, EPI_RESID_SPLIT, splits, 0, wpb, parts=parts, counters=cnt, resid=residual, ssp=ssp,
                     ar=tp)
    return ssp


_RESID_CAP = {}


def skinny_resid_capacity(N: Optional[int] = None) -> int:
    for waves in (4, 8):
        if waves not in _RESID_CAP:
            _RESID_CAP[waves] = int(_fn("mrsum_skinny_resid_capacity_w")(waves))
    return min(_RESID_CAP[4], _RESID_CAP[8])


def skinny_resid(x: torch.Tensor, w, residual: torch.Tensor, tp=None) -> torch.Tensor:
    N = w.shape[0]
    fp8 = isinstance(w, Fp8Weight)
    M = x.shape[0]
    ssp = torch.empty(M, N // 16, dtype=torch.float32, device=x.device)
    if tp is not None:
        cap = skinny_fp8_resid_capacity() if fp8 else skinny_resid_capacity(N)
        _req(N // 16 <= cap, "skinny_resid: TP-push grid of %d workgroups is not fully resident (capacity %d)"
             % (N // 16, cap))
        STATS["tp_push"] += 1
    if fp8:
        _skinny_fp8(x, w, None, EPI_SKINNY_RESID, 1, 1, 0, resid=residual, ssp=ssp, ar=tp)
    else:
        _skinny(x, w, None, EPI_SKINNY_RESID, 1, 1, 0, resid=residual, ssp=ssp, ar=tp)
    return ssp


def skinny_fp8_resid_capacity() -> int:
    if "fp8" not in _RESID_CAP:
        _RESID_CAP["fp8"] = int(_fn("mrsum_skinny_fp8_resid_capacity")())
    return _RESID_CAP["fp8"]


def linear_swiglu(x: torch.Tensor, w_gu: torch.Tensor, out: Optional[torch.Tensor] = None,
                  kernel: str = "skinny", wpb: int = 4, splits: int = 1, norm=None) -> torch.Tensor:
    M = x.shape[0]
    F2 = w_gu.shape[0]
    _req(norm is None or kernel in ("stream", "stream_split", "skinny"),
         "linear_swiglu: a deferred norm needs the stream or register-streaming kernel")
    if kernel == "gemm" or M > (STREAM_MAX_M_SWIGLU if kernel == "stream" else SKINNY_MAX_M):
        return gemm(x, w_gu, out=out, swiglu=True)
    if out is None:
        out = torch.empty(M, F2 // 2, dtype=x.dtype, device=x.device)
    _req(out.is_contiguous() and out.shape == (M, F2 // 2), "linear_swiglu: bad out")
    if kernel == "stream":
        return _stream_gemm(x, w_gu, out, EPI_SWIGLU, 1, F2 // 2, wpb, norm=norm)
    if kernel == "stream_split":
        return stream_swiglu_split(x, w_gu, out, wpb, splits, norm=norm)
    if kernel == "lds":
        return _skinny_lds(x, w_gu, out, EPI_SWIGLU, 1, F2 // 2)
    return _skinny(x, w_gu, out, EPI_SWIGLU, 1, 1, F2 // 2, norm=norm)


def add_rmsnorm_parts(parts: torch.Tensor, residual: torch.Tensor, w: torch.Tensor, eps: float,
                      out: Optional[torch.Tensor] = None) -> torch.Tensor:
    _req(parts.is_cuda and parts.dtype == torch.float32 and parts.is_contiguous() and parts.dim() == 3,
         "add_rmsnorm_parts: parts must be fp32 [S, T, D]")
    _bf16_cuda(residual, w)
    S, T, D = parts.shape
    _req(residual.shape == (T, D) and residual.is_contiguous() and w.numel() == D and D % 8 == 0,
         "add_rmsnorm_parts: shapes")
    if out is None:
        out = torch.empty(T, D, dtype=residual.dtype, device=residual.device)
    _rows_ok(out)
    _check(_fn("mrsum_add_rmsnorm_parts")(_p(parts), S, _p(residual), _p(w), _p(out), T, D, out.stride(0), eps,
                                          _stream()), "add_rmsnorm_parts")
    return out


N_CU = 256
STATS = {"tp_push": 0}


def stream_config(N: int, K: int, swiglu: bool = False, splits: Optional[int] = None, max_splits: int = 16):
    if K % 128:
        return None
    nkb = K // 128
    best, best_key = None, None
    for wpb in (4, 5, 6, 7, 8):
        if N % (16 * wpb):
            continue
        tiles = N // (16 * wpb)
        cands = [1] if swiglu else ([splits] if splits else range(1, max_splits + 1))
        for S in cands:
            if nkb % S:
# ... 256 lines not shown
```

Before: 2.191.

## Fuse LM-head GEMM with sampling in persistent kernel; fuse embed+rmsnorm; prefill GEMM path

Adds a persistent streaming GEMM for large-N skinny projections like the LM head. One variant computes per-row Gumbel-max sample keys in the epilogue and writes per-workgroup maxima to a slab, which a new finish kernel reduces, so full logits are never written out or reread. It also adds a fused embedding gather plus RMSNorm kernel and routes prefill projections and SwiGLU through the dense GEMM path. These cut logits memory traffic, kernel launches and per-tile scheduling overhead, at the cost of more code paths and a different sampling reduction order.

```diff
diff --git a/llm_map_reduce_summarizer_amd/csrc/kernels/norm.hip b/llm_map_reduce_summarizer_amd/csrc/kernels/norm.hip
--- a/llm_map_reduce_summarizer_amd/csrc/kernels/norm.hip
+++ b/llm_map_reduce_summarizer_amd/csrc/kernels/norm.hip
@@ -1,15 +1,22 @@
 #include "common.h"
 
-template <int VPT, bool ADD, int Q8 = 0>
+template <int VPT, bool ADD, int Q8 = 0, bool EMBED = false>
 __global__ __launch_bounds__(256) void rmsnorm_kernel(const bf16* __restrict__ x, bf16* __restrict__ residual,
                                                       const bf16* __restrict__ w, bf16* __restrict__ out,
                                                       int D, int x_stride, int out_stride, float eps,
-                                                      float* __restrict__ qscale = nullptr) {
+                                                      float* __restrict__ qscale = nullptr,
+                                                      const int* __restrict__ ids = nullptr, int V = 0) {
+    static_assert(!(ADD && EMBED), "the gathered row is the residual");
     __shared__ float red[16];
     const int row = blockIdx.x;
     const int nvec = D >> 3;
-    const uint4* xr = reinterpret_cast<const uint4*>(x + (size_t)row * x_stride);
-    uint4* rr = ADD ? reinterpret_cast<uint4*>(residual + (size_t)row * D) : nullptr;
+    int src = row;
+    if constexpr (EMBED) {
+        src = ids[row];
+        src = src < 0 ? 0 : (src >= V ? V - 1 : src);
+    }
+    const uint4* xr = reinterpret_cast<const uint4*>(x + (size_t)src * x_stride);
+    uint4* rr = ADD || EMBED ? reinterpret_cast<uint4*>(residual + (size_t)row * D) : nullptr;
     float v[VPT][8];
     const uint4* wr = reinterpret_cast<const uint4*>(w);
     uint4 wv[VPT];
@@ -20,7 +27,9 @@
     for (int i = 0; i < VPT; ++i) {
         const int c = threadIdx.x + i * 256;
         if (c < nvec) {
-            unpack8(xr[c], v[i]);
+            const uint4 xv = xr[c];
+            unpack8(xv, v[i]);
+            if constexpr (EMBED) rr[c] = xv;
             if (ADD) {
                 float r[8];
                 unpack8(rr[c], r);
@@ -124,6 +133,22 @@
     return launch_rmsnorm<false>(x, nullptr, w, out, T, D, x_stride, out_stride, eps, s);
 }
 
+MRSUM_API int mrsum_embed_rmsnorm(const int* ids, const void* table, const void* w, void* residual, void* out, int T,
+                                  int D, int V, float eps, hipStream_t s) {
+    if (T <= 0) return 0;
+    if (D % 8 || D > 256 * 8 * 8 || V <= 0) return (int)hipErrorInvalidValue;
+    const int vpt = ceil_div(D / 8, 256);
+    dim3 g(T), b(256);
+    auto X = (const bf16*)table; auto R = (bf16*)residual; auto W = (const bf16*)w; auto O = (bf16*)out;
+#define LE(VPT_) rmsnorm_kernel<VPT_, false, 0, true><<<g, b, 0, s>>>(X, R, W, O, D, D, D, eps, nullptr, ids, V)
+    if (vpt <= 1) LE(1);
+    else if (vpt <= 2) LE(2);
+    else if (vpt <= 4) LE(4);
+    else LE(8);
+#undef LE
+    return (int)hipGetLastError();
+}
+
 MRSUM_API int mrsum_add_rmsnorm(const void* x, void* residual, const void* w, void* out, int T, int D,
                                 int x_stride, int out_stride, float eps, hipStream_t s) {
     return launch_rmsnorm<true>(x, residual, w, out, T, D, x_stride, out_stride, eps, s);
diff --git a/llm_map_reduce_summarizer_amd/csrc/kernels/sample_key.h b/llm_map_reduce_summarizer_amd/csrc/kernels/sample_key.h
--- /dev/null
+++ b/llm_map_reduce_summarizer_amd/csrc/kernels/sample_key.h
@@ -0,0 +1,30 @@
+#pragma once
+#include "common.h"
+
+__device__ __forceinline__ unsigned long long mix64(unsigned long long x) {
+    x ^= x >> 30; x *= 0xbf58476d1ce4e5b9ULL;
+    x ^= x >> 27; x *= 0x94d049bb133111ebULL;
+    x ^= x >> 31;
+    return x;
+}
+
+__device__ __forceinline__ unsigned int order_key(float v) {
+    const unsigned int b = __float_as_uint(v);
+    return (b & 0x80000000u) ? ~b : (b | 0x80000000u);
+}
+
+__device__ __forceinline__ unsigned long long sample_key0(long long seed, int position) {
+    return mix64((unsigned long long)seed * 0x9E3779B97F4A7C15ULL + (unsigned long long)(position + 1));
+}
+
+__device__ __forceinline__ float sample_inv_tau(float tau) { return tau > 0.f ? 1.f / tau : 0.f; }
+
+__device__ __forceinline__ unsigned long long sample_key(float v, int tok, float tau, float inv_tau,
+                                                         unsigned long long key0) {
+    if (tau > 0.f) {
+        const unsigned long long h = mix64(key0 ^ ((unsigned long long)tok * 0xD1B54A32D192ED03ULL));
+        const float u = ((float)(h >> 40) + 0.5f) * (1.f / 16777216.f);
+        v = v * inv_tau - __logf(-__logf(u));
+    }
+    return ((unsigned long long)order_key(v) << 32) | (unsigned long long)(0xFFFFFFFFu - (unsigned int)tok);
+}
diff --git a/llm_map_reduce_summarizer_amd/csrc/kernels/sampler.hip b/llm_map_reduce_summarizer_amd/csrc/kernels/sampler.hip
--- a/llm_map_reduce_summarizer_amd/csrc/kernels/sampler.hip
+++ b/llm_map_reduce_summarizer_amd/csrc/kernels/sampler.hip
@@ -1,18 +1,6 @@
-#include "common.h"
+#include "sample_key.h"
 
 constexpr int EOS_SLOTS = 4;
-
-__device__ __forceinline__ unsigned long long mix64(unsigned long long x) {
-    x ^= x >> 30; x *= 0xbf58476d1ce4e5b9ULL;
-    x ^= x >> 27; x *= 0x94d049bb133111ebULL;
-    x ^= x >> 31;
-    return x;
-}
-
-__device__ __forceinline__ unsigned int order_key(float v) {
-    const unsigned int b = __float_as_uint(v);
-    return (b & 0x80000000u) ? ~b : (b | 0x80000000u);
-}
 
 constexpr int FILTER_BINS = 65536;
 constexpr int FILTER_R = 4;
@@ -221,9 +209,8 @@
     const float tau = temps[b];
     float th = -INFINITY;
     if constexpr (FILTER) th = thresh[b];
-    const float inv_tau = tau > 0.f ? 1.f / tau : 0.f;
-    const unsigned long long key0 =
-        mix64((unsigned long long)seeds[b] * 0x9E3779B97F4A7C15ULL + (unsigned long long)(positions[b] + 1));
+    const float inv_tau = sample_inv_tau(tau);
+    const unsigned long long key0 = sample_key0(seeds[b], positions[b]);
     const int c0 = blockIdx.x * seg_len;
     const int c1 = min(V, c0 + seg_len);
     const bf16* row = logits + (size_t)b * ld;
@@ -239,17 +226,11 @@
 #pragma unroll
         for (int j = 0; j < 8; ++j) {
             const int tok = tok_offset + c + j;
-            float v = f[j];
+            const float v = f[j];
             if constexpr (FILTER) {
                 if (v < th) continue;
             }
-            if (tau > 0.f) {
-                const unsigned long long h = mix64(key0 ^ ((unsigned long long)tok * 0xD1B54A32D192ED03ULL));
-                const float u = ((float)(h >> 40) + 0.5f) * (1.f / 16777216.f);
-                v = v * inv_tau - __logf(-__logf(u));
-            }
-            const unsigned long long k =
-                ((unsigned long long)order_key(v) << 32) | (unsigned long long)(0xFFFFFFFFu - (unsigned int)tok);
+            const unsigned long long k = sample_key(v, tok, tau, inv_tau, key0);
             if (c + j < c1 && k > best) best = k;
         }
     }
@@ -267,14 +248,33 @@
     }
 }
 
+template <bool SLAB>
 __global__ void sample_finish_kernel(unsigned long long* __restrict__ result, int* __restrict__ next_ids,
                                      int* __restrict__ positions, int* __restrict__ gen_count,
                                      const int* __restrict__ max_new, int* __restrict__ out_tokens, int out_stride,
-                                     int* __restrict__ done, const int* __restrict__ eos, int B) {
-    const int b = blockIdx.x * blockDim.x + threadIdx.x;
-    if (b >= B) return;
-    const unsigned long long r = result[b];
-    result[b] = 0ULL;
+                                     int* __restrict__ done, const int* __restrict__ eos, int B,
+                                     const unsigned long long* __restrict__ slab = nullptr, int G = 0) {
+    int b;
+    unsigned long long r;
+    if constexpr (SLAB) {
+        b = blockIdx.x;
+        r = 0ULL;
+        for (int i = threadIdx.x; i < G; i += 64) {
+            const unsigned long long k = slab[(size_t)i * B + b];
+            r = k > r ? k : r;
+        }
+#pragma unroll
+        for (int o = 32; o > 0; o >>= 1) {
+            const unsigned long long other = __shfl_xor(r, o, 64);
+            r = other > r ? other : r;
+        }
+        if (threadIdx.x != 0) return;
+    } else {
+        b = blockIdx.x * blockDim.x + threadIdx.x;
+        if (b >= B) return;
+        r = result[b];
+        result[b] = 0ULL;
+    }
     if (done[b]) return;
     const int tok = (int)(0xFFFFFFFFu - (unsigned int)(r & 0xFFFFFFFFULL));
     const int g = gen_count[b];
@@ -308,8 +308,18 @@
                                   int* out_tokens, int out_stride, int* done, const int* eos, int B,
                                   hipStream_t s) {
     if (B <= 0) return 0;
-    sample_finish_kernel<<<ceil_div(B, 64), 64, 0, s>>>((unsigned long long*)result, next_ids, positions_rw,
+    sample_finish_kernel<false><<<ceil_div(B, 64), 64, 0, s>>>((unsigned long long*)result, next_ids, positions_rw,
                                                         gen_count, max_new, out_tokens, out_stride, done, eos, B);
+    return (int)hipGetLastError();
+}
+
+MRSUM_API int mrsum_sample_finish_slab(const void* slab, int G, int* next_ids, int* positions_rw, int* gen_count,
+                                       const int* max_new, int* out_tokens, int out_stride, int* done,
+                                       const int* eos, int B, hipStream_t s) {
+    if (B <= 0) return 0;
+    if (G <= 0 || !slab) return (int)hipErrorInvalidValue;
+    sample_finish_kernel<true><<<B, 64, 0, s>>>(nullptr, next_ids, positions_rw, gen_count, max_new, out_tokens,
+                                               out_stride, done, eos, B, (const unsigned long long*)slab, G);
     return (int)hipGetLastError();
 }
 
@@ -320,7 +330,7 @@
     if (B <= 0) return 0;
     int e = launch_keys(logits, ld, B, V, 0, temps, seeds, positions, result, s);
     if (e) return e;
-    sample_finish_kernel<<<ceil_div(B, 64), 64, 0, s>>>((unsigned long long*)result, next_ids, positions_rw,
+    sample_finish_kernel<false><<<ceil_div(B, 64), 64, 0, s>>>((unsigned long long*)result, next_ids, positions_rw,
                                                         gen_count, max_new, out_tokens, out_stride, done, eos, B);
     return (int)hipGetLastError();
 }
@@ -352,7 +362,7 @@
                                                       (unsigned long long*)result, seg_len, thresh);
     e = (int)hipGetLastError();
     if (e) return e;
-    sample_finish_kernel<<<ceil_div(B, 64), 64, 0, s>>>((unsigned long long*)result, next_ids, positions_rw,
+    sample_finish_kernel<false><<<ceil_div(B, 64), 64, 0, s>>>((unsigned long long*)result, next_ids, positions_rw,
                                                         gen_count, max_new, out_tokens, out_stride, done, eos, B);
     return (int)hipGetLastError();
 }
diff --git a/llm_map_reduce_summarizer_amd/csrc/kernels/stream_gemm.hip b/llm_map_reduce_summarizer_amd/csrc/kernels/stream_gemm.hip
--- a/llm_map_reduce_summarizer_amd/csrc/kernels/stream_gemm.hip
+++ b/llm_map_reduce_summarizer_amd/csrc/kernels/stream_gemm.hip
@@ -1,4 +1,5 @@
 #include "ar_common.h"
+#include "sample_key.h"
 
 namespace {
 enum { EPI_BF16 = 0, EPI_F32_PARTIAL = 1, EPI_SWIGLU = 2, EPI_SWIGLU_SPLIT = 3, EPI_RESID_SPLIT = 4 };
@@ -429,6 +430,219 @@
 #undef BY_WPB
 #undef L
     return (int)hipGetLastError();
+}
+
+struct SampleArgs {
+    const float* temps;
+    const long long* seeds;
+    const int* positions;
+    unsigned long long* slab;
+};
+
+template <int MT, int WPB, bool NTW, bool SAMPLE>
+__global__ __launch_bounds__(64 * WPB, 1) void stream_persist_kernel(const bf16* __restrict__ x, int ldx,
+                                                                     const bf16* __restrict__ W, int K, int M,
+                                                                     bf16* __restrict__ out, int ldo, int tiles,
+                                                                     const NormArgs e, const SampleArgs sa) {
+    constexpr int R = 16 * WPB, BM = 16 * MT;
+    constexpr int WBYTES = R * 256, SLOT = WBYTES + BM * 256;
+    constexpr int D = (LDS_BUDGET / SLOT) < 6 ? (LDS_BUDGET / SLOT) : 6;
+    static_assert(D >= 3, "ring too shallow");
+    constexpr int XP = 2 * BM / 8;
+    constexpr int XI = (XP + WPB - 1) / WPB;
+    constexpr int NI = 4 + XI;
+    __shared__ __attribute__((aligned(1024))) char lds[D * SLOT + LDS_XTRA];
+    float* const s_ss = reinterpret_cast<float*>(lds + D * SLOT + 1024);
+
+    const int tid = threadIdx.x, lane = tid & 63, w = tid >> 6;
+    const int G = gridDim.x, b = blockIdx.x;
+    const int cnt = tiles / G + (b < tiles % G ? 1 : 0);
+    const int t0 = b * (tiles / G) + min(b, tiles % G);
+    const int nkb = K / KBLK;
+    const int T = cnt * nkb;
+
+    const int prow = lane >> 3, pslot = lane & 7;
+    const bf16* wsrc[4];
+#pragma unroll
+    for (int p = 0; p < 4; ++p) {
+        const int q = 4 * w + p;
+        const int row = 8 * (q >> 1) + prow;
+        wsrc[p] = W + ((size_t)t0 * R + row) * K + 8 * (8 * (q & 1) + (pslot ^ prow));
+    }
+    const bf16* xsrc[XI];
+    int xdst[XI];
+#pragma unroll
+    for (int i = 0; i < XI; ++i) {
+        const int q = w + WPB * i;
+        const int qq = q < XP ? q : 0;
+        const int row = 8 * (qq >> 1) + prow;
+        xsrc[i] = x + (size_t)min(row, M - 1) * ldx + 8 * (8 * (qq & 1) + (pslot ^ prow));
+        xdst[i] = q < XP ? WBYTES + q * 1024 : -1;
+    }
+    int ikb = 0, inext = 1;
+    size_t woff = 0;
+    const size_t tile_step = (size_t)R * K - (size_t)(K - KBLK);
+#define ISSUE_P(slot)                                                                                \
+    {                                                                                                \
+        char* base = lds + (slot) * SLOT;                                                            \
+        _Pragma("unroll") for (int p = 0; p < 4; ++p) glds16<NTW ? 2 : 0>(wsrc[p] + woff, base + (4 * w + p) * 1024); \
+        _Pragma("unroll") for (int i = 0; i < XI; ++i)                                               \
+            glds16(xsrc[i] + ikb * KBLK, xdst[i] >= 0 ? base + xdst[i] : lds + D * SLOT);            \
+        if (inext < T) {   \
+            ++inext;                                                                                 \
+            if (++ikb == nkb) { ikb = 0; woff += tile_step; } else woff += KBLK;                     \
+        }                                                                                            \
+    }
+
+#pragma unroll
+    for (int s = 0; s < D - 1; ++s) ISSUE_P(s);
+
+    const int r = lane & 15, g = lane >> 4;
+    float sc[MT];
+#pragma unroll
+    for (int m = 0; m < MT; ++m) sc[m] = 1.f;
+    if (e.ssq) {
+        row_norm_partials(e, M, tid, 64 * WPB, s_ss);
+        __syncthreads();
+#pragma unroll
+        for (int m = 0; m < MT; ++m) sc[m] = row_scale(e, s_ss, min(16 * m + r, M - 1));
+    }
+    float tau[MT], inv_tau[MT];
+    unsigned long long key0[MT], best[MT];
+    if constexpr (SAMPLE) {
+#pragma unroll
+        for (int m = 0; m < MT; ++m) {
+            const int mm = min(16 * m + r, M - 1);
+            tau[m] = sa.temps[mm];
+            inv_tau[m] = sample_inv_tau(tau[m]);
+            key0[m] = sample_key0(sa.seeds[mm], sa.positions[mm]);
+            best[m] = 0ULL;
+        }
+    }
+
+    int f = 0, slot = 0, fslot = D - 1;
+    for (int t = 0; t < cnt; ++t) {
+        f32x4 acc[MT];
+#pragma unroll
+        for (int m = 0; m < MT; ++m) acc[m] = f32x4{0.f, 0.f, 0.f, 0.f};
+        for (int j = 0; j < nkb; ++j, ++f) {
+            if (f + D - 2 < T) wait_vmcnt<NI * (D - 2)>();
+            else wait_vmcnt<0>();
+            raw_barrier();
+            if (f + D - 1 < T) {
+                ISSUE_P(fslot);
+                fslot = fslot + 1 == D ? 0 : fslot + 1;
+            }
+            const char* wl = lds + slot * SLOT;
+            const char* xl = wl + WBYTES;
+            slot = slot + 1 == D ? 0 : slot + 1;
+#pragma unroll
+            for (int i = 0; i < 4; ++i) {
+                const u32x4 av = *reinterpret_cast<const u32x4*>(wl + img_off(16 * w + r, 4 * i + g));
+#pragma unroll
+                for (int m = 0; m < MT; ++m) {
+                    const u32x4 bv = *reinterpret_cast<const u32x4*>(xl + img_off(16 * m + r, 4 * i + g));
+                    acc[m] = __builtin_amdgcn_mfma_f32_16x16x32_bf16(__builtin_bit_cast(bf16x8, av),
+                                                                     __builtin_bit_cast(bf16x8, bv), acc[m], 0, 0, 0);
+                }
+            }
+        }
+        const int nw = (t0 + t) * R + 16 * w;
+#pragma unroll
+        for (int m = 0; m < MT; ++m) {
+            const int mm = 16 * m + r;
+            if (e.ssq) { acc[m][0] *= sc[m]; acc[m][1] *= sc[m]; acc[m][2] *= sc[m]; acc[m][3] *= sc[m]; }
+            if (mm < M) {
+                uint2 o;
+                o.x = pack2(acc[m][0], acc[m][1]);
+                o.y = pack2(acc[m][2], acc[m][3]);
+                if constexpr (SAMPLE) {
+                    const float v[4] = {__uint_as_float(o.x << 16), __uint_as_float(o.x & 0xffff0000u),
+                                        __uint_as_float(o.y << 16), __uint_as_float(o.y & 0xffff0000u)};
+#pragma unroll
+                    for (int jj = 0; jj < 4; ++jj) {
+                        const unsigned long long k = sample_key(v[jj], nw + 4 * g + jj, tau[m], inv_tau[m], key0[m]);
+                        best[m] = k > best[m] ? k : best[m];
+                    }
+                } else {
+                    *reinterpret_cast<uint2*>(out + (size_t)mm * ldo + nw + 4 * g) = o;
+                }
+            }
+        }
+    }
+#undef ISSUE_P
+    if constexpr (SAMPLE) {
+        unsigned long long* s_best = reinterpret_cast<unsigned long long*>(lds);
+        __syncthreads();
+#pragma unroll
+        for (int m = 0; m < MT; ++m) {
+            unsigned long long k = best[m];
+#pragma unroll
+            for (int o = 16; o <= 32; o <<= 1) {
+                const unsigned long long other = __shfl_xor(k, o, 64);
+                k = other > k ? other : k;
+            }
+            if (g == 0) s_best[64 * w + 16 * m + r] = k;
+        }
+        __syncthreads();
+        if (tid < M) {
+            unsigned long long k = s_best[tid];
+#pragma unroll
+            for (int i = 1; i < WPB; ++i) k = s_best[64 * i + tid] > k ? s_best[64 * i + tid] : k;
+            sa.slab[(size_t)blockIdx.x * M + tid] = k;
+        }
+    }
+}
+
+template <bool SAMPLE>
+static int launch_persist(const void* x, int ldx, const void* W, int N, int K, int M, void* out, int ldo, int wpb,
+                          int max_wgs, const float* ssq, int ssq_tiles, float eps, const SampleArgs sa,
+                          hipStream_t s) {
+    if (M <= 0) return 0;
+    if (wpb < 4 || wpb > 8 || M > 64 || K % KBLK || K < KBLK || N % (16 * wpb) || N <= 0 || max_wgs < 1 || ldo < N ||
+        ldo % 4)
+        return (int)hipErrorInvalidValue;
+    if (ssq && (ssq_tiles <= 0 || ssq_tiles % (4 * SS_PARTS))) return (int)hipErrorInvalidValue;
+    NormArgs e = {};
+    e.ssq = ssq; e.ssq_tiles = ssq_tiles; e.inv_k = 1.f / (float)K; e.eps = eps;
+    const int tiles = N / (16 * wpb);
+    const int mt = (M + 15) / 16;
+    dim3 grid(tiles < max_wgs ? tiles : max_wgs), block(64 * wpb);
+    auto X = (const bf16*)x;
+    auto Wp = (const bf16*)W;
+#define LP(MT_, WPB_) \
+    stream_persist_kernel<MT_, WPB_, true, SAMPLE><<<grid, block, 0, s>>>(X, ldx, Wp, K, M, (bf16*)out, ldo, tiles, e, sa)
+#define BY_WPB_P(MT_)                        \
+    switch (wpb) {                           \
+        case 4: LP(MT_, 4); break;           \
+        case 5: LP(MT_, 5); break;           \
+        case 6: LP(MT_, 6); break;           \
+        case 7: LP(MT_, 7); break;           \
+        default: LP(MT_, 8); break;          \
+    }
+    switch (mt) {
+        case 1: BY_WPB_P(1); break;
+        case 2: BY_WPB_P(2); break;
+        case 3: BY_WPB_P(3); break;
+        default: BY_WPB_P(4); break;
+    }
+#undef BY_WPB_P
+#undef LP
+    return (int)hipGetLastError();
+}
+
+MRSUM_API int mrsum_stream_persist(const void* x, int ldx, const void* W, int N, int K, int M, void* out, int ldo,
+                                   int wpb, int max_wgs, const float* ssq, int ssq_tiles, float eps, hipStream_t s) {
+    if (!out) return (int)hipErrorInvalidValue;
+    return launch_persist<false>(x, ldx, W, N, K, M, out, ldo, wpb, max_wgs, ssq, ssq_tiles, eps, SampleArgs{}, s);
+}
+
+MRSUM_API int mrsum_stream_persist_sample(const void* x, int ldx, const void* W, int N, int K, int M, int wpb,
+                                          int max_wgs, const float* ssq, int ssq_tiles, float eps, const float* temps,
+                                          const long long* seeds, const int* positions, void* slab, hipStream_t s) {
+    if (!temps || !seeds || !positions || !slab) return (int)hipErrorInvalidValue;
+    return launch_persist<true>(x, ldx, W, N, K, M, nullptr, N, wpb, max_wgs, ssq, ssq_tiles, eps,
+                                SampleArgs{temps, seeds, positions, (unsigned long long*)slab}, s);
 }
 
 namespace {
diff --git a/llm_map_reduce_summarizer_amd/engine/engine.py b/llm_map_reduce_summarizer_amd/engine/engine.py
--- a/llm_map_reduce_summarizer_amd/engine/engine.py
+++ b/llm_map_reduce_summarizer_amd/engine/engine.py
@@ -368,12 +368,14 @@
 
     def _decode_once(self, B: int, filtered: bool = False) -> None:
         st = self.state
+        v = st.view(0, B)
+        v.filtered = filtered
+        fused = not filtered and not self.model.tp_sampling
         logits = self.model.decode(st.next_ids[:B], st.positions[:B], st.seq_idx[:B], st.block_tables[:B],
                                    self.kv.k, self.kv.v, workspace=self._workspace(B),
-                                   gather=filtered or not self.model.tp_sampling)
-        v = st.view(0, B)
-        v.filtered = filtered
-        self._sample(logits, v)
+                                   gather=filtered or not self.model.tp_sampling, sample=v if fused else None)
+        if logits is not None:
+            self._sample(logits, v)
 
     def _decode_steps(self, B: int, steps: int, filtered: bool = False) -> None:
         if filtered:
diff --git a/llm_map_reduce_summarizer_amd/engine/model.py b/llm_map_reduce_summarizer_amd/engine/model.py
--- a/llm_map_reduce_summarizer_amd/engine/model.py
+++ b/llm_map_reduce_summarizer_amd/engine/model.py
@@ -63,6 +63,10 @@
 
 
 _QKV_SPLIT = os.environ.get("MRSUM_FP8_QKV_SPLIT", "1") == "1"
+
+
+PREFILL_TRIM = os.environ.get("MRSUM_PREFILL_TRIM", "1") == "1"
+KEEP_NONE = object()
 
 
 def _hip():
@@ -293,23 +297,39 @@
 
     def run_layers(self, ids: torch.Tensor, positions: torch.Tensor, seq_idx: torch.Tensor,
                    block_tables: torch.Tensor, kcache: torch.Tensor, vcache: torch.Tensor,
-                   attention: Callable[[int, torch.Tensor], torch.Tensor], decode: bool = False) -> torch.Tensor:
+                   attention: Callable[[int, torch.Tensor], torch.Tensor], decode: bool = False,
+                   keep=None) -> Optional[torch.Tensor]:
         c = self.cfg
-        residual = ops.embed(ids, self.embed)
         q8 = not decode and self.weight_dtype == "fp8"
         q8qkv = ("split" if _QKV_SPLIT else True) if q8 else False
-        x = ops.rmsnorm(residual, None, c.rms_eps, quant=q8qkv)
+        if q8:
+            residual = ops.embed(ids, self.embed)
+            x = ops.rmsnorm(residual, None, c.rms_eps, quant=q8qkv)
+        else:
+            residual, x = ops.embed_rmsnorm(ids, self.embed, c.rms_eps)
         page = _page_of(kcache, self.hd)
         ar = _TPReduce(self) if self.tp_size > 1 else (LocalReduce(self) if self.emulate_tp_reduce else None)
         last = len(self.layers) - 1
+        trim = keep is not None and PREFILL_TRIM and not decode
         for i, lw in enumerate(self.layers):
             qkv = ops.qkv_rope(x, lw.wqkv, positions, seq_idx, block_tables, kcache[i], vcache[i], self.cos_sin,
                                self.hq, self.hkv, self.hd, page, defer=decode)
+            if i == last and trim and keep is KEEP_NONE:
+                return None
             a = attention(i, qkv)
+            if i == last and trim and keep is not KEEP_NONE and ar is None and self._trim_ok(a, lw):
+                a, residual = a.index_select(0, keep), residual.index_select(0, keep)
+                x = ops.proj_add_rmsnorm(a, lw.wo, residual, None, c.rms_eps, "o", None, quant=q8, prefill=True)
+                return ops.mlp(x, lw.wgu, lw.wdown, residual, c.rms_eps, None, quant=False, prefill=True)
             x = ops.proj_add_rmsnorm(a, lw.wo, residual, None, c.rms_eps, "o", ar, quant=q8)
             x = ops.mlp(x, lw.wgu, lw.wdown, residual, c.rms_eps, ar,
                         quant=q8qkv if i < last else False)
-        return x
+        if keep is KEEP_NONE:
+            return None
+        return x if keep is None else ops.rows(x).index_select(0, keep)
+
+    def _trim_ok(self, a: torch.Tensor, lw: LayerWeights) -> bool:
+        return a.is_cuda and all(ops.prefill_rows(a.shape[0], w.shape[1]) for w in (lw.wo, lw.wgu, lw.wdown))
 
     def logits(self, x: torch.Tensor, gather: bool = True) -> torch.Tensor:
         local = ops.linear(x, self.lm_head)
@@ -327,10 +347,11 @@
             pp = paged.layer(kcache[i], vcache[i]) if paged is not None else None
             return ops.attn_prefill(qkv, cu_seqlens, self.hq, self.hkv, self.hd, self.scale, paged=pp, **kw)
 
-        x = self.run_layers(ids, positions, seq_idx, block_tables, kcache, vcache, attention)
+        x = self.run_layers(ids, positions, seq_idx, block_tables, kcache, vcache, attention,
+                            keep=last_rows if logits else KEEP_NONE)
         if not logits:
             return None
-        return self.logits(ops.rows(x).index_select(0, last_rows), gather)
+        return self.logits(x, gather)
 
     def prefill_passes(self, passes, block_tables: torch.Tensor, kcache: torch.Tensor, vcache: torch.Tensor,
                        gather: bool = True) -> torch.Tensor:
@@ -418,7 +439,8 @@
         return self.logits(ops.rows(s["x"]).index_select(0, p.last_rows))
 
     def decode(self, ids: torch.Tensor, positions: torch.Tensor, seq_idx: torch.Tensor, block_tables: torch.Tensor,
-               kcache: torch.Tensor, vcache: torch.Tensor, workspace=None, gather: bool = True) -> torch.Tensor:
+               kcache: torch.Tensor, vcache: torch.Tensor, workspace=None, gather: bool = True,
+               sample=None) -> Optional[torch.Tensor]:
         page = _page_of(kcache, self.hd)
 
         def attention(i, qkv):
@@ -426,4 +448,7 @@
                                    page, self.scale, workspace=workspace)
 
         x = self.run_layers(ids, positions, seq_idx, block_tables, kcache, vcache, attention, decode=True)
+        if sample is not None and self.tp_size == 1 and ops.lm_head_samples(x, self.lm_head):
+            ops.lm_head_sample(x, self.lm_head, sample)
+            return None
         return self.logits(x, gather)
diff --git a/llm_map_reduce_summarizer_amd/ops/__init__.py b/llm_map_reduce_summarizer_amd/ops/__init__.py
--- a/llm_map_reduce_summarizer_amd/ops/__init__.py
+++ b/llm_map_reduce_summarizer_amd/ops/__init__.py
@@ -143,6 +143,14 @@
     return _impl(table).embed(ids, table, out)
 
 
+def embed_rmsnorm(ids, table, eps):
+    if _use_hip(table):
+        from . import hip
+        return hip.embed_rmsnorm(ids, table, unit_gain(table.shape[1], table.device), eps)
+    residual = reference.embed(ids, table)
+    return residual, reference.rmsnorm(residual, unit_gain(table.shape[1], table.device), eps)
+
+
 class PagedPrefill:
 
     def __init__(self, block_tables, seq_slot, prefix, slot_host, prefix_host, kcache=None, vcache=None):
@@ -187,6 +195,21 @@
         thresh = st.thresh[:n]
     toks = reference.sample_tokens(logits, st.temps[:n], st.seeds[:n], st.positions[:n], thresh)
     reference.sample_finish(toks, st)
+
+
+def lm_head_samples(x, lm_head) -> bool:
+    xt = x.h if isinstance(x, NormRows) else x
+    if not _use_hip(xt) or isinstance(lm_head, Fp8Weight):
+        return False
+    from . import hip
+    return hip.lm_head_sample_cfg(xt.shape[0], lm_head.shape[0], xt.shape[1]) is not None
+
+
+def lm_head_sample(x, lm_head, st):
+    from . import hip
+    if isinstance(x, NormRows):
+        return hip.lm_head_sample(x.h, lm_head, st, norm=x.norm)
+    return hip.lm_head_sample(x, lm_head, st)
 
 
 def sample_tp(logits, st, tok_offset, max_reduce):
@@ -333,7 +356,22 @@
     return ("stream",) + tuple(cfg)
 
 
-def proj_add_rmsnorm(a, w, residual, ln, eps, role="o", all_reduce=None, quant=False):
+def prefill_rows(T, K):
+    from . import hip
+    return T > max(hip.STREAM_MAX_M, hip.STREAM_MAX_M_SWIGLU) and K % 128 == 0
+
+
+def proj_add_rmsnorm(a, w, residual, ln, eps, role="o", all_reduce=None, quant=False, prefill=False):
+    if prefill and _use_hip(a):
+        from . import hip
+        if ln is None:
+            ln = unit_gain(residual.shape[1], residual.device)
+        o = hip.gemm_fp8(*hip.quant_fp8_rows(a), w) if isinstance(w, Fp8Weight) else hip.gemm(a, w)
+        if all_reduce:
+            all_reduce(o)
+        if quant and o.shape[1] % 16 == 0:
+            return QuantRows(*hip.rmsnorm_fp8(o, ln, eps, residual=residual, split=quant == "split"))
+        return hip.add_rmsnorm(o, residual, ln, eps)
     if _use_hip(a):
         from . import hip
         if ln is None and a.shape[0] <= hip.SKINNY_MAX_M:
@@ -391,12 +429,19 @@
     return reference.add_rmsnorm(o, residual, ln, eps)
 
 
-def mlp(x, wgu, wdown, residual, eps, all_reduce=None, quant=False):
-    act = gate_up_swiglu(x, wgu)
-    return proj_add_rmsnorm(act, wdown, residual, None, eps, "down", all_reduce, quant=quant)
-
-
-def gate_up_swiglu(x, wgu):
+def mlp(x, wgu, wdown, residual, eps, all_reduce=None, quant=False, prefill=False):
+    act = gate_up_swiglu(x, wgu, prefill=prefill)
+    return proj_add_rmsnorm(act, wdown, residual, None, eps, "down", all_reduce, quant=quant, prefill=prefill)
+
+
+def gate_up_swiglu(x, wgu, prefill=False):
+    if prefill and (isinstance(x, QuantRows) or _use_hip(x)):
+        from . import hip
+        if isinstance(x, QuantRows):
+            return hip.gemm_fp8(x.q, x.scale, wgu, swiglu=True)
+        if isinstance(wgu, Fp8Weight):
+            return hip.gemm_fp8(*hip.quant_fp8_rows(x), wgu, swiglu=True)
+        return hip.gemm(x, wgu, swiglu=True)
     if isinstance(x, QuantRows):
         from . import hip
         return hip.fp8_linear_swiglu(x.pair, wgu)
diff --git a/llm_map_reduce_summarizer_amd/ops/hip.py b/llm_map_reduce_summarizer_amd/ops/hip.py
--- a/llm_map_reduce_summarizer_amd/ops/hip.py
+++ b/llm_map_reduce_summarizer_amd/ops/hip.py
@@ -37,6 +37,12 @@
     "mrsum_skinny_lds": [_vp, _c_int, _vp, _c_int, _c_int, _c_int, _vp, _c_int, _c_int, _c_int, _c_int, _vp],
     "mrsum_stream_gemm": [_vp, _c_int, _vp, _c_int, _c_int, _c_int, _vp, _c_int, _c_int, _c_int, _c_int, _vp, _vp,
                           _vp, _c_int, _c_float, _vp, _c_int, _vp, _c_int, _vp, _vp],
+    "mrsum_stream_persist": [_vp, _c_int, _vp, _c_int, _c_int, _c_int, _vp, _c_int, _c_int, _c_int, _vp, _c_int,
+                             _c_float, _vp],
+    "mrsum_stream_persist_sample": [_vp, _c_int, _vp, _c_int, _c_int, _c_int, _c_int, _c_int, _vp, _c_int, _c_float,
+                                    _vp, _vp, _vp, _vp, _vp],
+    "mrsum_sample_finish_slab": [_vp, _c_int, _vp, _vp, _vp, _vp, _vp, _c_int, _vp, _vp, _c_int, _vp],
+    "mrsum_embed_rmsnorm": [_vp, _vp, _vp, _vp, _vp, _c_int, _c_int, _c_int, _c_float, _vp],
     "mrsum_stream_fp8": [_vp, _c_int, _vp, _vp, _c_int, _c_int, _c_int, _vp, _c_int, _c_int, _c_int, _c_int, _vp, _vp,
                          _vp, _c_int, _c_float, _vp, _c_int, _vp, _vp, _vp],
     "mrsum_skinny_fp8": [_vp, _c_int, _vp, _vp, _c_int, _c_int, _c_int, _vp, _c_int, _c_int, _c_int, _c_int, _vp,
@@ -260,6 +266,20 @@
     _req(out.is_contiguous() and out.shape == (T, D), "embed: bad out")
     _check(_fn("mrsum_embed")(_p(ids), _p(table), _p(out), T, D, V, _stream()), "embed")
     return out
+
+
+def embed_rmsnorm(ids: torch.Tensor, table: torch.Tensor, w: torch.Tensor, eps: float):
+    _i32(ids)
+    _bf16_cuda(table, w)
+    V, D = table.shape
+    _req(table.is_contiguous() and w.numel() == D and w.is_contiguous() and D % 8 == 0 and D <= 16384,
+         "embed_rmsnorm: table must be [V, D] contiguous, D % 8 == 0, D <= 16384")
+    T = ids.numel()
+    residual = torch.empty(T, D, dtype=table.dtype, device=table.device)
+    out = torch.empty(T, D, dtype=table.dtype, device=table.device)
+    _check(_fn("mrsum_embed_rmsnorm")(_p(ids), _p(table), _p(w), _p(residual), _p(out), T, D, V, eps, _stream()),
+           "embed_rmsnorm")
+    return residual, out
 
 
 def prefill_block_m(group: int) -> int:
@@ -761,6 +781,79 @@
     return out
 
 
+LM_HEAD_PERSIST = os.environ.get("MRSUM_LM_HEAD_PERSIST", "1") == "1"
+
+
+_CU_COUNT = {}
+
+
+def cu_count(device) -> int:
+    key = str(device)
+    if key not in _CU_COUNT:
+        _CU_COUNT[key] = int(torch.cuda.get_device_properties(device).multi_processor_count)
+    return _CU_COUNT[key]
+
+
+def persist_cfg(M: int, N: int, K: int):
+    if not (1 <= M <= SKINNY_MAX_M) or K % 128 or not LM_HEAD_PERSIST:
+        return None
+    cfg = stream_config(N, K, splits=1)
+    if cfg is None or N // (16 * cfg[0]) <= N_CU:
+        return None
+    return cfg[0]
+
+
+def stream_persist(x: torch.Tensor, w: torch.Tensor, out: torch.Tensor, wpb: int, norm=None,
+                   max_wgs: Optional[int] = None) -> torch.Tensor:
+    _bf16_cuda(x, w, out)
+    _rows_ok(x)
+    M, K = x.shape
+    N = w.shape[0]
+    max_wgs = cu_count(x.device) if max_wgs is None else int(max_wgs)
+    _req(w.is_contiguous() and w.shape[1] == K, "stream_persist: weight must be [N, K] contiguous")
+    _req(1 <= M <= SKINNY_MAX_M and K % 128 == 0 and K >= 128 and 4 <= wpb <= 8 and N % (16 * wpb) == 0
+         and max_wgs >= 1, "stream_persist: unsupported shape M=%d N=%d K=%d wpb=%d" % (M, N, K, wpb))
+    _req(out.is_contiguous() and out.shape == (M, N), "stream_persist: bad out")
+    sq, tiles, eps = _norm_args(x, norm)
+    _check(_fn("mrsum_stream_persist")(_p(x), x.stride(0), _p(w), N, K, M, _p(out), N, wpb, max_wgs, sq, tiles, eps,
+                                       _stream()), "stream_persist")
+    return out
+
+
+LM_HEAD_SAMPLE = os.environ.get("MRSUM_LM_HEAD_SAMPLE", "1") == "1"
+
+
+def lm_head_sample_cfg(M: int, N: int, K: int):
+    return persist_cfg(M, N, K) if LM_HEAD_SAMPLE else None
+
+
+def lm_head_sample(x: torch.Tensor, w: torch.Tensor, st, norm=None, wpb: Optional[int] = None,
+                   max_wgs: Optional[int] = None) -> None:
+    _bf16_cuda(x, w)
+    _rows_ok(x)
+    M, K = x.shape
+    N = w.shape[0]
+    wpb = persist_cfg(M, N, K) if wpb is None else wpb
+    max_wgs = cu_count(x.device) if max_wgs is None else int(max_wgs)
+    _req(wpb is not None and w.is_contiguous() and w.shape[1] == K and 1 <= M <= SKINNY_MAX_M and K % 128 == 0
+         and 4 <= wpb <= 8 and N % (16 * wpb) == 0 and max_wgs >= 1,
+         "lm_head_sample: unsupported shape M=%d N=%d K=%d" % (M, N, K))
+    _req(st.temps.numel() >= M and st.seeds.numel() >= M and st.positions.numel() >= M and st.next_ids.numel() >= M
+         and st.out_tokens.shape[0] >= M and st.temps.dtype == torch.float32 and st.seeds.dtype == torch.int64
+         and st.temps.is_cuda and st.seeds.is_cuda, "lm_head_sample: state smaller than batch")
+    _i32(st.positions, st.next_ids, st.gen_count, st.max_new, st.done)
+    _eos_ok(st)
+    G = min(N // (16 * wpb), max_wgs)
+    slab = torch.empty(G, M, dtype=torch.int64, device=x.device)
+    sq, tiles, eps = _norm_args(x, norm)
+    _check(_fn("mrsum_stream_persist_sample")(_p(x), x.stride(0), _p(w), N, K, M, wpb, max_wgs, sq, tiles, eps,
+                                              _p(st.temps), _p(st.seeds), _p(st.positions), _p(slab), _stream()),
+           "stream_persist_sample")
+    _check(_fn("mrsum_sample_finish_slab")(_p(slab), G, _p(st.next_ids), _p(st.positions), _p(st.gen_count),
+                                           _p(st.max_new), _p(st.out_tokens), st.out_tokens.stride(0), _p(st.done),
+                                           _p(st.eos), M, _stream()), "sample_finish_slab")
+
+
 def linear_takes_norm(M: int, N: int, K: int) -> bool:
     return 1 <= M <= SKINNY_MAX_M and K % 128 == 0 and stream_config(N, K, splits=1) is not None
 
@@ -778,6 +871,9 @@
     _req(out.is_contiguous() and out.shape == (M, N), "linear: bad out")
     if tall:
         return _stream_gemm(x, w, out, EPI_BF16, 1, N, tall_wpb(N, M, 1))
+    pw = persist_cfg(M, N, K)
+    if pw is not None:
+        return stream_persist(x, w, out, pw, norm=norm)
     cfg = stream_config(N, K, splits=1)
     if cfg is not None:
         return _stream_gemm(x, w, out, EPI_BF16, 1, N, cfg[0], norm=norm)
```

Result: no change. 2.204 (median of 6 runs) (+0.6%).
